# Fabri000/Maze-Solving-Agent-Gymnasium

Measured on NVIDIA B200. Metric: env-steps/sec (40x40 mazes, whole job), higher is better.
Workload: dtype u8/int32 state+obs, f64 reward

## Files before the change

include/maze_b200.h:

```cpp
#ifndef MAZE_B200_H
#define MAZE_B200_H

#include <stdint.h>

#ifdef __cplusplus
extern "C" {
#endif

#define MAZE_ABI_VERSION 12

#define MAZE_E_NULL   (-1)
#define MAZE_E_RANGE  (-2)
#define MAZE_E_SHAPE  (-3)
#define MAZE_E_ALGO   (-4)
#define MAZE_E_ALIGN  (-5)

#define MAZE_MAX_DIM      255
#define MAZE_GEN_MAX_DIM  131
#define MAZE_GEN_MAX_CELLS 64
#define MAZE_WINDOW       15

#define MAZE_ALGO_RPRIM     0
#define MAZE_ALGO_DFS       1
#define MAZE_ALGO_PRIMKILL  2

#define MAZE_META_WORDS 8
#define MAZE_META_H          0
#define MAZE_META_W          1
#define MAZE_META_START      2
#define MAZE_META_GOAL       3
#define MAZE_META_MAX_STEPS  4
#define MAZE_META_FLAGS      5
#define MAZE_META_SOL_LEN    6
#define MAZE_META_SPARE      7
#define MAZE_FLAG_TOROIDAL 1

#define MAZE_TAB_OPEN      0x01
#define MAZE_TAB_CODE_SHIFT 1
#define MAZE_TAB_D4_SHIFT   4

#define MAZE_ST_NEEDS_RESET 0x01
#define MAZE_ST_WON         0x02
#define MAZE_ST_MOVE_SHIFT  2
#define MAZE_ST_NMOVES_SHIFT 4

#define MAZE_STEP_AUTORESET   0x01
#define MAZE_STEP_WIN_NEXT    0x02
#define MAZE_STEP_WIN_QUEUE   0x04
#define MAZE_STEP_PACKED      0x08
#define MAZE_STEP_NO_WIDE     0x10

#define MAZE_REC_CODE_SHIFT   16
#define MAZE_REC_TERM_SHIFT   19
#define MAZE_REC_TRUNC_SHIFT  20
#define MAZE_REC_KIND_SHIFT   21
#define MAZE_REC_INDEX_SHIFT  23
#define MAZE_REC_KIND_REVISIT 0
#define MAZE_REC_KIND_INVALID 1
#define MAZE_REC_KIND_SHAPING 2
#define MAZE_REC_KIND_CONST   3
#define MAZE_REC_CONST_ZERO      0
#define MAZE_REC_CONST_ONE       1
#define MAZE_REC_CONST_MINUS_ONE 2
#define MAZE_REC_REWARD(kind, index) (((uint32_t)(kind) << MAZE_REC_KIND_SHIFT) | ((uint32_t)(index) << MAZE_REC_INDEX_SHIFT))

typedef struct maze_ctx maze_ctx;

typedef struct maze_env_batch {
    int32_t   num_envs;
    int32_t   num_mazes;
    int32_t   slot;
    int32_t   pool_stride;
    const int32_t* meta;
    const uint8_t* table;
    int32_t*  env_maze;
    uint64_t* state;
    uint16_t* visits;
    int32_t*  agent;
    int32_t*  target;
    int32_t*  best_dir;
    double*   reward;
    uint8_t*  terminated;
    uint8_t*  truncated;
    double*   ep_return;
    int64_t*  stats;
    double*   stats_return;
    int32_t*  queue;
    int32_t*  queue_count;
    int64_t   visit_cell_stride;
    int64_t   visit_env_stride;
    int32_t   visit_tiled;
    int32_t   visit_slot;
    int32_t*  target_dirty;
    uint32_t* packed;
    uint32_t* visit_bits;
    int32_t   visit_bits_pitch;
    int32_t   visit_bits_stride;
    int32_t   flags;
    int32_t   reserved;
} maze_env_batch;
#define MAZE_BATCH_BORDERED 1

int  maze_sizeof(int which);

int  maze_abi_version(void);
int  maze_ctx_create(maze_ctx** out, int device);
void maze_ctx_destroy(maze_ctx* ctx);
const char* maze_last_error(maze_ctx* ctx);

int maze_reward_lut(maze_ctx* ctx, int kind, double* out);

int maze_fields(maze_ctx* ctx, const uint8_t* grids, int32_t* meta, uint8_t* table,
                const int32_t* ids, int n, int slot, void* stream);

int maze_step(maze_ctx* ctx, const maze_env_batch* b, const uint8_t* actions, uint32_t mode, void* stream);

int maze_step_decode_host(const uint32_t* records, int64_t n, const int32_t* shape, const uint8_t* toroidal, int32_t* agent,
                          int32_t* best_dir, double* reward, uint8_t* terminated, uint8_t* truncated);

int maze_bench_scatter_rmw(maze_ctx* ctx, const maze_env_batch* b, const uint8_t* actions, uint16_t* arr, int64_t n_elems, int pattern,
                           int rmw_per_1024, uint32_t launch, int streams, void* stream);

typedef struct maze_step_trace {
    int32_t* agent;
    int32_t* best_dir;
    double*  reward;
    uint8_t* terminated;
    uint8_t* truncated;
} maze_step_trace;
int maze_step_many(maze_ctx* ctx, const maze_env_batch* b, const uint8_t* actions, int k_steps, uint32_t mode,
                   const maze_step_trace* trace, int chunk_envs, void* stream);

int maze_reset(maze_ctx* ctx, const maze_env_batch* b, const uint8_t* mask, void* stream);

int maze_generate(maze_ctx* ctx, uint8_t* grids, int32_t* meta, uint8_t* table, const int32_t* ids,
                  const int32_t* count_dev, int n, int slot, int max_h, int max_w,
                  uint64_t seed, int64_t slot_id_base, int candidates, double* difficulty, void* stream);

int maze_curriculum(maze_ctx* ctx, int32_t* meta, int32_t* wins, const int32_t* ids, const int32_t* count_dev,
                    int n, int grow, int max_h, int max_w, int wins_a, int algo_a, int wins_b, int algo_b, void* stream);

int maze_regen_swap(maze_ctx* ctx, uint8_t* grids, uint8_t* table, int32_t* meta, const uint8_t* shadow_grids, const uint8_t* shadow_table,
                    const int32_t* shadow_meta, const int32_t* ready_gen, int depth, const int32_t* queue, const int32_t* queue_count, int n,
                    int slot, int32_t* refill_queue, int32_t* refill_count, int32_t* queued_tag, int batch, int32_t* slow_queue,
                    int32_t* slow_count, int32_t* stats, int32_t* wins, void* stream);
int maze_regen_prepare(maze_ctx* ctx, const int32_t* meta, const int32_t* base_meta, const int32_t* base_wins, int grow, int max_h, int max_w,
                       int wins_a, int algo_a, int wins_b, int algo_b, int32_t* shadow_meta, int32_t* ready_gen, int depth,
                       const int32_t* refill_queue, const int32_t* refill_count, int n, int32_t* work_queue, int32_t* work_count, void* stream);
int maze_regen_publish(maze_ctx* ctx, const int32_t* shadow_meta, int32_t* ready_gen, int depth, const int32_t* work_queue,
                       const int32_t* work_count, int n, void* stream);

int maze_window(maze_ctx* ctx, const maze_env_batch* b, float* window, double* agent_norm, double* target_norm,
                void* stream);

int maze_direction_mask(maze_ctx* ctx, const maze_env_batch* b, int probs, float* mask, void* stream);

#define MAZE_Q_EMPTY     0xffffffffffffffffull
#define MAZE_Q_NO_SLOT   0xffffffffu
typedef struct maze_q_agent {
    int64_t   capacity;
    uint64_t* keys;
    double*   q_a;
    double*   q_b;
    int32_t*  overflow;
    int32_t   envs_per_agent;
    int32_t   eps_len;
    const double* eps_lut;
    double*   gamma;
    double    lr;
    double    eta;
    uint32_t* slot;
    uint32_t* steps_done;
    uint8_t*  last_action;
    double*   ep_return;
    uint64_t  seed;
    int64_t   env_id_base;
    const double*  u_tape;
    const uint8_t* a_tape;
    uint32_t* tape_pos;
    int32_t   u_len, a_len;
} maze_q_agent;

int maze_q_epsilon_lut(double initial_epsilon, double final_epsilon, double decay, double* out, int n);

int maze_q_act(maze_ctx* ctx, const maze_env_batch* b, const maze_q_agent* agent, uint8_t* actions, void* stream);

int maze_q_update(maze_ctx* ctx, const maze_env_batch* b, const maze_q_agent* agent, void* stream);

int maze_q_rollout(maze_ctx* ctx, const maze_env_batch* b, const maze_q_agent* agent, int k_steps, uint32_t mode,
                   void* stream);

#define MAZE_WINDOW_WORDS 24
typedef struct maze_replay {
    int64_t   capacity;
    unsigned long long* pushed;
    float*    vec;
    float*    next_vec;
    uint32_t* win;
    uint32_t* next_win;
    uint8_t*  action;
    float*    reward;
    float*    stage_vec;
    uint32_t* stage_win;
    int32_t   without_replacement;
    int32_t   reserved;
} maze_replay;

int maze_dqn_observe(maze_ctx* ctx, const maze_env_batch* b, const maze_replay* r, void* stream);

int maze_dqn_push(maze_ctx* ctx, const maze_env_batch* b, const maze_replay* r, const uint8_t* actions, void* stream);

int maze_dqn_sample(maze_ctx* ctx, const maze_replay* r, int n, uint64_t seed, uint64_t draw, float* vec, float* win,
                    float* next_vec, float* next_win, int64_t* action, float* reward, void* stream);

int maze_dqn_select(maze_ctx* ctx, const maze_env_batch* b, const float* q_values, const double* eps_lut, int eps_len,
                    uint32_t* steps_done, uint64_t seed, int64_t env_id_base, uint8_t* actions, void* stream);

#define MAZE_NET_IN       1600
#define MAZE_NET_IN_USED  1574
#define MAZE_NET_H1       1024
#define MAZE_NET_H2       512
#define MAZE_NET_OFF_CONV_W 0
#define MAZE_NET_OFF_CONV_B 864
#define MAZE_NET_OFF_W1     896
#define MAZE_NET_OFF_B1     (MAZE_NET_OFF_W1 + MAZE_NET_H1 * MAZE_NET_IN)
#define MAZE_NET_OFF_W2     (MAZE_NET_OFF_B1 + MAZE_NET_H1)
#define MAZE_NET_OFF_B2     (MAZE_NET_OFF_W2 + MAZE_NET_H2 * MAZE_NET_H1)
#define MAZE_NET_OFF_W3     (MAZE_NET_OFF_B2 + MAZE_NET_H2)
#define MAZE_NET_OFF_B3     (MAZE_NET_OFF_W3 + 4 * MAZE_NET_H2)
#define MAZE_NET_PARAMS     (MAZE_NET_OFF_B3 + 4)
typedef struct maze_dqn_net {
    float*    params;
    float*    target;
    float*    grads;
    float*    adam_m;
    float*    adam_v;
    uint16_t* w1_bf16;
    uint16_t* w2_bf16;
    uint16_t* w1t_bf16;
    uint16_t* w2t_bf16;
    uint16_t* tw1_bf16;
    uint16_t* tw2_bf16;
    void*     workspace;
    float*    loss;
    int32_t   max_batch;
    int32_t   reserved;
} maze_dqn_net;

int64_t maze_dqn_net_workspace_bytes(int max_batch);

int maze_dqn_net_refresh(maze_ctx* ctx, const maze_dqn_net* net, int which, void* stream);

int maze_dqn_forward(maze_ctx* ctx, const maze_dqn_net* net, int which, const float* vec, const uint32_t* win, int n,
                     float* q_out, void* stream);

int maze_dqn_features(maze_ctx* ctx, const maze_dqn_net* net, int which, const float* vec, const uint32_t* win, int n,
                      uint16_t* X, uint8_t* pool_idx, void* stream);

int maze_dqn_backward(maze_ctx* ctx, const maze_dqn_net* net, const float* vec, const uint32_t* win, const float* next_vec,
                      const uint32_t* next_win, const uint8_t* action, const float* reward, int n, float gamma,
                      float* qsa_out, void* fc_ready_event, void* stream);

int maze_dqn_adamw(maze_ctx* ctx, const maze_dqn_net* net, float lr, float beta1, float beta2, float eps, float weight_decay,
                   int64_t step, float grad_scale, float clamp, void* stream);

int maze_dqn_net_profile(maze_ctx* ctx, int enable);
int maze_dqn_net_profile_read(maze_ctx* ctx, float* ms, char* labels, int label_bytes, int cap, int* count);

int maze_dqn_sample_packed(maze_ctx* ctx, const maze_replay* r, int n, uint64_t seed, uint64_t draw, float* vec, uint32_t* win,
                           float* next_vec, uint32_t* next_win, uint8_t* action, float* reward, void* stream);

int maze_dqn_gemm_bf16(maze_ctx* ctx, const uint16_t* A, int lda, const uint16_t* B, int ldb, void* C, int ldc, int M, int N, int K,
                       int epilogue, int act, const float* bias, const uint16_t* aux, int ldaux, int tile_n, int splits, void* stream);

#define MAZE_METRIC_WORDS 8
#define MAZE_METRIC_DIFFICULTY 0
#define MAZE_METRIC_COMPLEXITY 1
#define MAZE_METRIC_L          2
#define MAZE_METRIC_DE         3
#define MAZE_METRIC_D          4
#define MAZE_METRIC_SOL_LEN    5
#define MAZE_METRIC_DE_COUNT   6
int maze_difficulty(maze_ctx* ctx, const uint8_t* grids, const int32_t* meta, const int32_t* ids,
                    int n, int slot, int max_h, int max_w, double* out, void* stream);

#define MAZE_METRIC_EXT_WORDS   20
#define MAZE_METRIC_EXT_DENSITY 0
#define MAZE_METRIC_EXT_T       1
#define MAZE_METRIC_EXT_J       2
#define MAZE_METRIC_EXT_CR      3
#define MAZE_METRIC_EXT_AC      4
#define MAZE_METRIC_EXT_FDE     5
#define MAZE_METRIC_EXT_BDE     6
#define MAZE_METRIC_EXT_L_DE    7
#define MAZE_METRIC_EXT_T_DE    8
#define MAZE_METRIC_EXT_D_SHARP 11
#define MAZE_METRIC_EXT_L_SHARP 14
int maze_difficulty_ext(maze_ctx* ctx, const uint8_t* grids, const int32_t* meta, const int32_t* ids,
                        int n, int slot, int max_h, int max_w, double* out, double* ext_out, void* stream);

#define MAZE_RENDER_TILE 16
int maze_render(maze_ctx* ctx, const maze_env_batch* b, const int32_t* env_ids, int n, uint8_t* out,
                int out_h, int out_w, void* stream);

#define MAZE_PACK_BITMAP 0
#define MAZE_PACK_WALLS  1
int maze_pack(maze_ctx* ctx, const uint8_t* grids, const int32_t* meta, const int32_t* ids, int n, int slot,
              int format, uint8_t* packed, int packed_stride, void* stream);
int maze_unpack(maze_ctx* ctx, const uint8_t* packed, int packed_stride, int format, uint8_t* grids,
                const int32_t* meta, const int32_t* ids, int n, int slot, void* stream);

int maze_collection_encode(maze_ctx* ctx, const uint8_t* grids, const int32_t* meta, const int32_t* ids, int n,
                           int slot, int h, int w, int32_t* out, void* stream);

#ifdef __cplusplus
}
#endif
#endif
```

maze-solving-agent-gymnasium_b200/csrc/maze_abi.cu:

```cuda
#include <cmath>
#include <cstdio>
#include <cstdlib>
#include <cstring>
#include <new>
#include "maze_common.cuh"

int maze_fail_cuda(maze_ctx* ctx, cudaError_t e, const char* what) {
    if (ctx) snprintf(ctx->err, sizeof(ctx->err), "CUDA error %d (%s) in %s", (int)e, cudaGetErrorString(e), what);
    return (int)e;
}

int maze_fail_arg(maze_ctx* ctx, int code, const char* what) {
    if (ctx) snprintf(ctx->err, sizeof(ctx->err), "argument error %d: %s", code, what);
    return code;
}

int maze_check_batch(maze_ctx* ctx, const maze_env_batch* b) {
    if (!b) return maze_fail_arg(ctx, MAZE_E_NULL, "batch");
    if (!b->meta || !b->table || !b->env_maze || !b->state || !b->visits || !b->agent || !b->target ||
        !b->best_dir || !b->reward || !b->terminated || !b->truncated)
        return maze_fail_arg(ctx, MAZE_E_NULL, "batch pointer");
    if (b->num_envs <= 0 || b->num_mazes <= 0 || b->slot <= 0 || (b->slot & 1))
        return maze_fail_arg(ctx, MAZE_E_RANGE, "num_envs / num_mazes / slot (must be even)");
    if (b->visit_slot < b->slot || (b->visit_tiled != 0 && b->visit_tiled != 1))
        return maze_fail_arg(ctx, MAZE_E_RANGE, "visit_slot (>= slot) / visit_tiled (0 or 1)");
    if (b->visit_bits && (b->visit_bits_pitch < 1 || b->visit_bits_stride < b->visit_bits_pitch || (b->visit_bits_stride & 3) ||
                          ((uintptr_t)b->visit_bits & 15)))
        return maze_fail_arg(ctx, MAZE_E_RANGE, "visit_bits: pitch >= 1, stride a multiple of 4 words, 16-byte aligned");
    if (b->visit_cell_stride <= 0 || b->visit_env_stride <= 0)
        return maze_fail_arg(ctx, MAZE_E_RANGE, "visit strides (cell-major: B, 1; env-major: 1, slot)");
    if (((uintptr_t)b->meta & 15) || ((uintptr_t)b->state & 7) || ((uintptr_t)b->agent & 7) ||
        ((uintptr_t)b->target & 7) || ((uintptr_t)b->best_dir & 7) || ((uintptr_t)b->reward & 7) ||
        ((uintptr_t)b->visits & 3))
        return maze_fail_arg(ctx, MAZE_E_ALIGN, "batch pointer alignment");
    return 0;
}


extern "C" int maze_abi_version(void) { return MAZE_ABI_VERSION; }

extern "C" int maze_sizeof(int which) {
    switch (which) {
        case 0: return (int)sizeof(maze_env_batch);
        case 1: return (int)sizeof(maze_q_agent);
        case 2: return (int)sizeof(maze_replay);
        case 3: return (int)sizeof(maze_step_trace);
        case 4: return (int)sizeof(maze_dqn_net);
        default: return -1;
    }
}

extern "C" int maze_ctx_create(maze_ctx** out, int device) {
    if (!out) return MAZE_E_NULL;
    *out = nullptr;
    maze_ctx* ctx = new (std::nothrow) maze_ctx();
    if (!ctx) return MAZE_E_RANGE;
    memset(ctx, 0, sizeof(*ctx));
    ctx->device = device;
    for (int i = 0; i < 256; ++i) {
        ctx->h_lut_revisit[i] = 0.0 - (1 - std::exp(-0.2 * i));
        ctx->h_lut_invalid[i] = 0.0 - (1 - std::exp(-0.15 * i));
    }
    ctx->h_shaping[0] = 0 * 0.5 - 0.05;
    ctx->h_shaping[1] = 1 * 0.5 - 0.05;
    ctx->h_shaping[2] = 0.0;
    ctx->h_shaping[3] = -1 * 0.5 - 0.05;
    cudaError_t e = cudaSetDevice(device);
    if (e == cudaSuccess) e = cudaMalloc(&ctx->d_lut_revisit, 256 * sizeof(double));
    if (e == cudaSuccess) e = cudaMalloc(&ctx->d_lut_invalid, 256 * sizeof(double));
    if (e == cudaSuccess) e = cudaMalloc(&ctx->d_counter, 4 * sizeof(int));
    if (e == cudaSuccess) e = cudaMemcpy(ctx->d_lut_revisit, ctx->h_lut_revisit, 256 * sizeof(double), cudaMemcpyHostToDevice);
    if (e == cudaSuccess) e = cudaMemcpy(ctx->d_lut_invalid, ctx->h_lut_invalid, 256 * sizeof(double), cudaMemcpyHostToDevice);
    if (e == cudaSuccess) e = cudaDeviceGetAttribute(&ctx->num_sms, cudaDevAttrMultiProcessorCount, device);
    if (e != cudaSuccess) {
        int rc = (int)e;
        cudaFree(ctx->d_lut_revisit);
        cudaFree(ctx->d_lut_invalid);
        cudaFree(ctx->d_counter);
        delete ctx;
        return rc;
    }
    ctx->step_ept = 2;
    if (const char* v = getenv("MAZE_STEP_EPT")) ctx->step_ept = atoi(v);
    if (const char* v = getenv("MAZE_L2_PERSIST_MB")) {
        int maxp = 0;
        cudaDeviceGetAttribute(&maxp, cudaDevAttrMaxPersistingL2CacheSize, device);
        size_t want = (size_t)atoi(v) << 20, before = 0, after = 0;
        if (want > (size_t)maxp) want = (size_t)maxp;
        cudaDeviceGetLimit(&before, cudaLimitPersistingL2CacheSize);
        cudaError_t le = cudaDeviceSetLimit(cudaLimitPersistingL2CacheSize, want);
        cudaDeviceGetLimit(&after, cudaLimitPersistingL2CacheSize);
        fprintf(stderr, "[maze_b200] persisting L2 %zu -> %zu bytes (max %d, rc %d)\n", before, after, maxp, (int)le);
    }
    if (const char* v = getenv("MAZE_L2_FETCH")) {
        size_t before = 0, after = 0;
        cudaDeviceGetLimit(&before, cudaLimitMaxL2FetchGranularity);
        cudaError_t le = cudaDeviceSetLimit(cudaLimitMaxL2FetchGranularity, (size_t)atoi(v));
        cudaDeviceGetLimit(&after, cudaLimitMaxL2FetchGranularity);
        fprintf(stderr, "[maze_b200] L2 fetch granularity %zu -> %zu (rc %d)\n", before, after, (int)le);
    }
    *out = ctx;
    return 0;
}

extern "C" void maze_ctx_destroy(maze_ctx* ctx) {
    if (!ctx) return;
    cudaFree(ctx->d_lut_revisit);
    cudaFree(ctx->d_lut_invalid);
    cudaFree(ctx->d_counter);
    cudaFree(ctx->d_scratch);
    maze_net_profile_free(ctx);
    delete ctx;
}

extern "C" const char* maze_last_error(maze_ctx* ctx) { return ctx ? ctx->err : "null ctx"; }

extern "C" int maze_reward_lut(maze_ctx* ctx, int kind, double* out) {
    if (!out) return MAZE_E_NULL;
    double rev[256], inv[256];
    for (int i = 0; i < 256; ++i) {
        rev[i] = 0.0 - (1 - std::exp(-0.2 * i));
        inv[i] = 0.0 - (1 - std::exp(-0.15 * i));
    }
    memset(out, 0, 256 * sizeof(double));
    if (kind == 0) memcpy(out, rev, sizeof(rev));
    else if (kind == 1) memcpy(out, inv, sizeof(inv));
    else if (kind == 2) { out[0] = -1 * 0.5 - 0.05; out[1] = 0 * 0.5 - 0.05; out[2] = 1 * 0.5 - 0.05; }
    else return maze_fail_arg(ctx, MAZE_E_RANGE, "maze_reward_lut kind");
    return 0;
}

extern "C" int maze_step_decode_host(const uint32_t* records, int64_t n, const int32_t* shape, const uint8_t* toroidal, int32_t* agent,
                                     int32_t* best_dir, double* reward, uint8_t* terminated, uint8_t* truncated) {
    if (!records || n < 0) return MAZE_E_NULL;
    double lut[4][256];
    memset(lut, 0, sizeof(lut));
    for (int i = 0; i < 256; ++i) {
        lut[MAZE_REC_KIND_REVISIT][i] = 0.0 - (1 - std::exp(-0.2 * i));
        lut[MAZE_REC_KIND_INVALID][i] = 0.0 - (1 - std::exp(-0.15 * i));
    }
    lut[MAZE_REC_KIND_SHAPING][0] = -1 * 0.5 - 0.05;
    lut[MAZE_REC_KIND_SHAPING][1] = 0 * 0.5 - 0.05;
    lut[MAZE_REC_KIND_SHAPING][2] = 1 * 0.5 - 0.05;
    lut[MAZE_REC_KIND_CONST][MAZE_REC_CONST_ONE] = 1.0;
    lut[MAZE_REC_KIND_CONST][MAZE_REC_CONST_MINUS_ONE] = -1.0;
    for (int64_t e = 0; e < n; ++e) {
        const uint32_t rec = records[e];
        const int r = (int)(rec & 0xff), c = (int)((rec >> 8) & 0xff), code = (int)((rec >> MAZE_REC_CODE_SHIFT) & 7);
        if (agent) { agent[2 * e] = r; agent[2 * e + 1] = c; }
        if (best_dir) {
            int br = 0, bc = 0;
            if (code < 4) {
                const int dr = (code == 0) - (code == 1), dc = (code == 2) - (code == 3);
                int nr = r + dr, nc = c + dc;
                if (toroidal && toroidal[e] && shape) {
                    const int H = shape[2 * e], W = shape[2 * e + 1];
                    nr = nr < 0 ? H - 1 : (nr >= H ? 0 : nr);
                    nc = nc < 0 ? W - 1 : (nc >= W ? 0 : nc);
                }
                br = r - nr;
                bc = c - nc;
            }
            best_dir[2 * e] = br;
            best_dir[2 * e + 1] = bc;
        }
        if (reward) reward[e] = lut[(rec >> MAZE_REC_KIND_SHIFT) & 3][(rec >> MAZE_REC_INDEX_SHIFT) & 0xff];
        if (terminated) terminated[e] = (uint8_t)((rec >> MAZE_REC_TERM_SHIFT) & 1);
        if (truncated) truncated[e] = (uint8_t)((rec >> MAZE_REC_TRUNC_SHIFT) & 1);
    }
    return 0;
}
```

maze-solving-agent-gymnasium_b200/csrc/maze_env.cuh:

```cuda
#pragma once
#include "maze_common.cuh"

struct StepLuts {
    const double* revisit;
    const double* invalid;
    double shaping_same, shaping_closer, shaping_farther;
};

inline StepLuts step_luts(const maze_ctx* ctx) {
    StepLuts l;
    l.revisit = ctx->d_lut_revisit;
    l.invalid = ctx->d_lut_invalid;
    l.shaping_same = ctx->h_shaping[0];
    l.shaping_closer = ctx->h_shaping[1];
    l.shaping_farther = ctx->h_shaping[3];
    return l;
}

#define VISIT_AT(b, e, idx) ((b).visits + (size_t)(idx) * (b).visit_cell_stride + (size_t)(e) * (b).visit_env_stride)

#ifndef MAZE_STATE_POLICY
#define MAZE_STATE_POLICY 1
#endif
#ifndef MAZE_TABLE_POLICY
#define MAZE_TABLE_POLICY 1
#endif
#ifndef MAZE_VISIT_POLICY
#define MAZE_VISIT_POLICY 1
#endif

template <int kPolicy>
__device__ __forceinline__ uint64_t l2_policy() {
    uint64_t p = 0;
    if (kPolicy == 1) asm volatile("createpolicy.fractional.L2::evict_last.b64 %0, 1.0;" : "=l"(p));
    if (kPolicy == 2) asm volatile("createpolicy.fractional.L2::evict_first.b64 %0, 1.0;" : "=l"(p));
    return p;
}
template <int kPolicy> __device__ __forceinline__ unsigned long long pol_load(const unsigned long long* p, uint64_t pol) {
    if (kPolicy == 0) return *p;
    unsigned long long v;
    asm volatile("ld.global.L2::cache_hint.u64 %0, [%1], %2;" : "=l"(v) : "l"(p), "l"(pol));
    return v;
}
template <int kPolicy> __device__ __forceinline__ int pol_load(const int* p, uint64_t pol) {
    if (kPolicy == 0) return *p;
    int v;
    asm volatile("ld.global.L2::cache_hint.s32 %0, [%1], %2;" : "=r"(v) : "l"(p), "l"(pol));
    return v;
}
template <int kPolicy> __device__ __forceinline__ unsigned pol_load(const uint16_t* p, uint64_t pol) {
    if (kPolicy == 0) return *p;
    unsigned short v;
    asm volatile("ld.global.L2::cache_hint.u16 %0, [%1], %2;" : "=h"(v) : "l"(p), "l"(pol));
    return v;
}
template <int kPolicy> __device__ __forceinline__ int pol_load_nc(const uint8_t* p, uint64_t pol) {
    if (kPolicy == 0) return __ldg(p);
    unsigned v;
    asm volatile("ld.global.nc.L2::cache_hint.u8 %0, [%1], %2;" : "=r"(v) : "l"(p), "l"(pol));
    return (int)v;
}
template <int kPolicy> __device__ __forceinline__ void pol_store(unsigned long long* p, unsigned long long v, uint64_t pol) {
    if (kPolicy == 0) { *p = v; return; }
    asm volatile("st.global.L2::cache_hint.u64 [%0], %1, %2;" ::"l"(p), "l"(v), "l"(pol) : "memory");
}
template <int kPolicy> __device__ __forceinline__ void pol_store(int* p, int v, uint64_t pol) {
    if (kPolicy == 0) { *p = v; return; }
    asm volatile("st.global.L2::cache_hint.s32 [%0], %1, %2;" ::"l"(p), "r"(v), "l"(pol) : "memory");
}
template <int kPolicy> __device__ __forceinline__ void pol_store(uint16_t* p, unsigned v, uint64_t pol) {
    if (kPolicy == 0) { *p = (uint16_t)v; return; }
    asm volatile("st.global.L2::cache_hint.u16 [%0], %1, %2;" ::"l"(p), "h"((unsigned short)v), "l"(pol) : "memory");
}
__device__ __forceinline__ unsigned visit_load(const uint16_t* p, uint64_t pol) { return pol_load<MAZE_VISIT_POLICY>(p, pol); }
#ifndef MAZE_VISIT_STORE_POLICY
#define MAZE_VISIT_STORE_POLICY MAZE_VISIT_POLICY
#endif
__device__ __forceinline__ void visit_store(uint16_t* p, unsigned v, uint64_t pol) {
    if (MAZE_VISIT_STORE_POLICY == MAZE_VISIT_POLICY) pol_store<MAZE_VISIT_POLICY>(p, v, pol);
    else pol_store<MAZE_VISIT_STORE_POLICY>(p, v, l2_policy<MAZE_VISIT_STORE_POLICY>());
}

__device__ __forceinline__ int visit_index(const maze_env_batch& b, int r, int c, int W) {
    if (b.visit_tiled) return (((r >> 2) * ((W + 3) >> 2) + (c >> 2)) << 4) | ((r & 3) << 2) | (c & 3);
    return r * W + c;
}

__device__ __forceinline__ void visit_bit_set(const maze_env_batch& b, int e, int r, int c) {
    if (b.visit_bits) atomicOr(b.visit_bits + (size_t)e * b.visit_bits_stride + r * b.visit_bits_pitch + (c >> 5), 1u << (c & 31));
}
__device__ __forceinline__ void visit_bits_clear(const maze_env_batch& b, int e) {
    if (!b.visit_bits) return;
    uint4* p = reinterpret_cast<uint4*>(b.visit_bits + (size_t)e * b.visit_bits_stride);
    for (int i = 0; i < (b.visit_bits_stride >> 2); ++i) p[i] = make_uint4(0, 0, 0, 0);
}

__device__ __forceinline__ void warp_clear_visits(unsigned need, const maze_env_batch& b, int e) {
    if (need & (1u << (threadIdx.x & 31)))
        for (int i = 0; i < b.visit_slot; ++i) *VISIT_AT(b, e, i) = 0;
}

__device__ __forceinline__ void begin_episode(EnvState& s, int start, int tab_at_start, bool& wrapped) {
    s.r = start & 0xffff;
    s.c = start >> 16;
    s.consec = 0;
    s.flags = 0;
    s.steps = 0;
    s.epoch += 1;
    wrapped = s.epoch > 255;
    if (wrapped) s.epoch = 1;
    s.tab = tab_at_start;
}

struct MazeView {
    int H, W, start, goal, max_steps;
    bool tor;
    const uint8_t* tab;
};

__device__ __forceinline__ MazeView load_maze(const maze_env_batch& b, int m) {
    const int4* mp = reinterpret_cast<const int4*>(b.meta + (size_t)m * MAZE_META_WORDS);
    const int4 m0 = __ldg(mp), m1 = __ldg(mp + 1);
    MazeView v;
    v.H = m0.x; v.W = m0.y; v.start = m0.z; v.goal = m0.w;
    v.max_steps = m1.x;
    v.tor = (m1.y & MAZE_FLAG_TOROIDAL) != 0;
    v.tab = b.table + (size_t)m * b.slot;
    return v;
}

struct StepResult {
    double reward;
    int term, trunc;
};

__device__ __forceinline__ StepResult env_transition(const maze_env_batch& b, int e, EnvState& st, const MazeView& mz,
                                                     int a, const StepLuts& luts) {
    StepResult out = {0.0, 0, 0};
    int dr, dc;
    action_delta(a, dr, dc);
    int nr = st.r + dr, nc = st.c + dc;
    bool inb = true;
    if (mz.tor) {
        nr = nr < 0 ? mz.H - 1 : (nr >= mz.H ? 0 : nr);
        nc = nc < 0 ? mz.W - 1 : (nc >= mz.W ? 0 : nc);
    } else {
        inb = (nr > 0) & (nr < mz.H - 1) & (nc > 0) & (nc < mz.W - 1);
    }
    const int idx = nr * mz.W + nc;
    const int tb = inb ? __ldg(mz.tab + idx) : 0;
    if (inb && (tb & MAZE_TAB_OPEN)) {
        const uint64_t pol = l2_policy<MAZE_VISIT_POLICY>();
        uint16_t* vp = VISIT_AT(b, e, visit_index(b, nr, nc, mz.W));
        const unsigned vis = visit_load(vp, pol);
        const int cnt = ((int)(vis >> 8) == st.epoch) ? (int)(vis & 0xff) : 0;
        if (cnt == 0) {
            if ((nr | (nc << 16)) == mz.goal) {
                out.reward = 1.0;
                out.term = 1;
            } else {
                const int dd = ((st.tab >> MAZE_TAB_D4_SHIFT) - (tb >> MAZE_TAB_D4_SHIFT)) & 3;
                out.reward = dd == 1 ? luts.shaping_closer : (dd == 3 ? luts.shaping_farther : luts.shaping_same);
            }
        } else {
            out.reward = __ldg(luts.revisit + cnt);
        }
        visit_store(vp, (unsigned)((st.epoch << 8) | (cnt < 255 ? cnt + 1 : 255)), pol);
        visit_bit_set(b, e, nr, nc);
        st.r = nr;
        st.c = nc;
        st.tab = tb;
        st.consec = 0;
        int nm = (st.flags >> MAZE_ST_NMOVES_SHIFT) & 3;
        nm = nm < 2 ? nm + 1 : 2;
        st.flags = (a << MAZE_ST_MOVE_SHIFT) | (nm << MAZE_ST_NMOVES_SHIFT);
    } else {
        st.consec = st.consec < 255 ? st.consec + 1 : 255;
        out.reward = __ldg(luts.invalid + st.consec);
        st.flags &= ~(MAZE_ST_NEEDS_RESET | MAZE_ST_WON);
    }
    st.steps = st.steps < 65535 ? st.steps + 1 : 65535;
    if (st.steps > mz.max_steps) {
        out.trunc = 1;
        out.reward = -1.0;
    }
    if (out.term | out.trunc) st.flags |= MAZE_ST_NEEDS_RESET | (out.term ? MAZE_ST_WON : 0);
    return out;
}
```

maze-solving-agent-gymnasium_b200/csrc/maze_obs.cu:

```cuda
#include "maze_env.cuh"
#include "maze_window.cuh"

namespace {

constexpr int OBS_THREADS = 256;
constexpr int WIN = MAZE_WINDOW;
constexpr int WIN_CELLS = WIN * WIN;

constexpr int WIN_ENVS = OBS_THREADS / 16;
constexpr int WIN_FLOATS = 3 * WIN_CELLS;

#ifndef MAZE_WIN_MINB
#define MAZE_WIN_MINB 4
#endif

__device__ __forceinline__ void window_row_to_smem(uint8_t* sl, unsigned m0, unsigned m1, unsigned m2) {
#pragma unroll
    for (int j = 0; j < WIN; ++j) {
        sl[j] = (uint8_t)((m0 >> j) & 1u);
        sl[WIN_CELLS + j] = (uint8_t)((m1 >> j) & 1u);
        sl[2 * WIN_CELLS + j] = (uint8_t)((m2 >> j) & 1u);
    }
}

__device__ __forceinline__ void window_norms(const EnvState& st, const MazeView& mz, int e, int hl, double* __restrict__ agent_norm,
                                             double* __restrict__ target_norm) {
    if (hl < 2) {
        const double shape = (double)(hl == 0 ? mz.H : mz.W);
        if (agent_norm) agent_norm[(size_t)e * 2 + hl] = __ddiv_rn((double)(hl == 0 ? st.r : st.c), shape);
        if (target_norm) target_norm[(size_t)e * 2 + hl] = __ddiv_rn((double)(hl == 0 ? (mz.goal & 0xffff) : (mz.goal >> 16)), shape);
    }
}

__device__ __forceinline__ void window_stream_out(const uint8_t* s_out, float* __restrict__ out, int n_float) {
    for (int q = threadIdx.x; 4 * q < n_float; q += OBS_THREADS) {
        const int f = 4 * q;
        const unsigned v = *reinterpret_cast<const unsigned*>(s_out + f);
        if (f + 3 < n_float) {
            __stcs(reinterpret_cast<float4*>(out) + q,
                   make_float4(__uint_as_float((v & 1u) * 0x3f800000u), __uint_as_float((v >> 8 & 1u) * 0x3f800000u),
                               __uint_as_float((v >> 16 & 1u) * 0x3f800000u), __uint_as_float((v >> 24 & 1u) * 0x3f800000u)));
        } else {
            for (int i = f; i < n_float; ++i) __stcs(out + i, (float)s_out[i]);
        }
    }
}

__global__ void __launch_bounds__(OBS_THREADS, MAZE_WIN_MINB)
maze_window_kernel(maze_env_batch b, float* __restrict__ window, double* __restrict__ agent_norm,
                   double* __restrict__ target_norm) {
    __shared__ __align__(16) uint8_t s_out[WIN_ENVS * WIN_FLOATS];
    const int hl = threadIdx.x & 15, w = threadIdx.x >> 4;
    const int e0 = blockIdx.x * WIN_ENVS, e = e0 + w;
    if (e < b.num_envs) {
        const EnvState st = unpack_state(b.state[e]);
        const MazeView mz = load_maze(b, b.env_maze[e]);
        unsigned m0, m1, m2;
        window_row_masks(b, e, st, mz, hl, m0, m1, m2);
        if (hl < WIN) window_row_to_smem(s_out + w * WIN_FLOATS + hl * WIN, m0, m1, m2);
        window_norms(st, mz, e, hl, agent_norm, target_norm);
    }
    __syncthreads();
    window_stream_out(s_out, window + (size_t)e0 * WIN_FLOATS, min(WIN_ENVS, b.num_envs - e0) * WIN_FLOATS);
}

constexpr int WINB_PER = 2;
constexpr int WINB_ENVS = WIN_ENVS * WINB_PER;

__global__ void __launch_bounds__(OBS_THREADS, MAZE_WIN_MINB)
maze_window_bordered_kernel(maze_env_batch b, float* __restrict__ window, double* __restrict__ agent_norm,
                            double* __restrict__ target_norm) {
    __shared__ __align__(16) uint8_t s_out[WINB_ENVS * WIN_FLOATS];
    const int hl = threadIdx.x & 15, w = threadIdx.x >> 4;
    const int e0 = blockIdx.x * WINB_ENVS;
    int e[WINB_PER];
    bool valid[WINB_PER];
    uint64_t raw[WINB_PER];
    int maze_id[WINB_PER];
#pragma unroll
    for (int u = 0; u < WINB_PER; ++u) {
        e[u] = e0 + w * WINB_PER + u;
        valid[u] = e[u] < b.num_envs;
        raw[u] = valid[u] ? b.state[e[u]] : 0ull;
        maze_id[u] = valid[u] ? b.env_maze[e[u]] : 0;
    }
    EnvState st[WINB_PER];
    MazeView mz[WINB_PER];
#pragma unroll
    for (int u = 0; u < WINB_PER; ++u) {
        st[u] = unpack_state(raw[u]);
        mz[u] = MazeView{};
        if (valid[u]) mz[u] = load_maze(b, maze_id[u]);
    }
    WindowRowRaw rows[WINB_PER];
    bool has[WINB_PER];
#pragma unroll
    for (int u = 0; u < WINB_PER; ++u) {
        has[u] = valid[u] && hl < WIN && mz[u].H >= WIN && mz[u].W >= WIN;
        rows[u] = WindowRowRaw{};
        if (has[u]) rows[u] = window_row_load_bits(b, e[u], st[u], mz[u], hl);
    }
#pragma unroll
    for (int u = 0; u < WINB_PER; ++u) {
        if (!valid[u]) continue;
        unsigned m0 = 0, m1 = 0, m2 = 0;
        if (has[u]) window_row_fold_bits(rows[u], mz[u], m0, m1, m2);
        if (hl < WIN) window_row_to_smem(s_out + (w * WINB_PER + u) * WIN_FLOATS + hl * WIN, m0, m1, m2);
        window_norms(st[u], mz[u], e[u], hl, agent_norm, target_norm);
    }
    __syncthreads();
    window_stream_out(s_out, window + (size_t)e0 * WIN_FLOATS, min(WINB_ENVS, b.num_envs - e0) * WIN_FLOATS);
}

__global__ void __launch_bounds__(OBS_THREADS)
maze_direction_mask_kernel(maze_env_batch b, int probs, float4* __restrict__ mask) {
    const int e = blockIdx.x * OBS_THREADS + threadIdx.x;
    if (e >= b.num_envs) return;
    const EnvState st = unpack_state(b.state[e]);
    const int m = b.env_maze[e];
    const int2 shape = __ldg(reinterpret_cast<const int2*>(b.meta + (size_t)m * MAZE_META_WORDS));
    const int H = shape.x, W = shape.y;
    const bool tor = (__ldg(b.meta + (size_t)m * MAZE_META_WORDS + MAZE_META_FLAGS) & MAZE_FLAG_TOROIDAL) != 0;
    const uint8_t* tab = b.table + (size_t)m * b.slot;
    float v[4];
#pragma unroll
    for (int a = 0; a < 4; ++a) {
        int dr, dc;
        action_delta(a, dr, dc);
        int nr = st.r + dr, nc = st.c + dc;
        bool open;
        if (tor) {
            nr = nr < 0 ? H - 1 : (nr >= H ? 0 : nr);
            nc = nc < 0 ? W - 1 : (nc >= W ? 0 : nc);
            open = (__ldg(tab + nr * W + nc) & MAZE_TAB_OPEN) != 0;
        } else {
            open = nr >= 0 && nr < H && nc >= 0 && nc < W && (__ldg(tab + nr * W + nc) & MAZE_TAB_OPEN) != 0;
        }
        v[a] = open ? 1.0f : 0.0f;
    }
    if (probs && ((st.flags >> MAZE_ST_NMOVES_SHIFT) & 3) >= 2) {
        const int last = (st.flags >> MAZE_ST_MOVE_SHIFT) & 3;
        const int back = tor ? 3 - last : (last ^ 1);
        v[back] = 0.25f;
    }
    mask[e] = make_float4(v[0], v[1], v[2], v[3]);
}

__global__ void __launch_bounds__(OBS_THREADS)
maze_render_kernel(maze_env_batch b, const int32_t* __restrict__ env_ids, int out_h, int out_w, uint8_t* __restrict__ out) {
    constexpr int T = MAZE_RENDER_TILE;
    const int k = blockIdx.x, r = blockIdx.y;
    const int e = env_ids ? env_ids[k] : k;
    const EnvState st = unpack_state(b.state[e]);
    const int m = b.env_maze[e];
    const int4 m0 = __ldg(reinterpret_cast<const int4*>(b.meta + (size_t)m * MAZE_META_WORDS));
    const int H = m0.x, W = m0.y;
    const int start_r = m0.z & 0xffff, start_c = m0.z >> 16, goal_r = m0.w & 0xffff, goal_c = m0.w >> 16;
    const uint8_t* tab = b.table + (size_t)m * b.slot;
    const bool has_moved = ((st.flags >> MAZE_ST_NMOVES_SHIFT) & 3) >= 1;
    __shared__ uint8_t s_tile[MAZE_GEN_MAX_DIM];
    for (int c = threadIdx.x; c < out_w / T; c += OBS_THREADS) {
        int code = 0;
        if (r < H && c < W) {
            const bool open = (__ldg(tab + r * W + c) & MAZE_TAB_OPEN) != 0;
            const int v = open ? ((r == goal_r && c == goal_c) ? 2 : 1) : 0;
            bool trail = false;
            if (open) {
                const unsigned vis = *VISIT_AT(b, e, visit_index(b, r, c, W));
                const int cnt = ((int)(vis >> 8) == st.epoch) ? (int)(vis & 0xff) : 0;
                if (r == start_r && c == start_c) trail = has_moved;
                else if (r == st.r && c == st.c) trail = cnt >= 2;
                else trail = cnt >= 1;
            }
            code = v | (trail ? 4 : 0) | 8;
        }
        s_tile[c] = (uint8_t)code;
    }
    __syncthreads();
    const int groups = out_w / 4;
    for (int p = threadIdx.x; p < T * groups; p += OBS_THREADS) {
        const int ly = p / groups, x0 = (p % groups) * 4, y = r * T + ly;
        if (y >= out_h) break;
        unsigned char px[12];
#pragma unroll
        for (int i = 0; i < 4; ++i) {
            const int x = x0 + i, c = x / T, lx = x % T;
            const int code = s_tile[c];
            int cr = 0, cg = 0, cb = 0;
            if ((code & 8) && x != W * T - 1 && y != H * T - 1) {
                const int v = code & 3;
                if (lx == 0 || lx == T - 1 || ly == 0 || ly == T - 1) {
                    if (code & 4) { cr = 208; cg = 135; cb = 112; } else { cr = 59; cg = 66; cb = 82; }
                } else if (r == st.r && c == st.c && lx >= T / 4 && lx < T / 4 + T / 2 && ly >= T / 4 && ly < T / 4 + T / 2) {
                    cr = 94; cg = 129; cb = 172;
                } else if (v == 0) { cr = 46; cg = 52; cb = 64; }
                else if (v == 1) { cr = 236; cg = 239; cb = 244; }
                else { cr = 163; cg = 190; cb = 140; }
            }
            px[3 * i] = (unsigned char)cr; px[3 * i + 1] = (unsigned char)cg; px[3 * i + 2] = (unsigned char)cb;
        }
        unsigned* o = reinterpret_cast<unsigned*>(out + (((size_t)k * out_h + y) * out_w + x0) * 3);
#pragma unroll
        for (int w = 0; w < 3; ++w)
            __stcs(o + w, (unsigned)px[4 * w] | ((unsigned)px[4 * w + 1] << 8) | ((unsigned)px[4 * w + 2] << 16) | ((unsigned)px[4 * w + 3] << 24));
    }
}

}

extern "C" int maze_render(maze_ctx* ctx, const maze_env_batch* b, const int32_t* env_ids, int n, uint8_t* out,
                           int out_h, int out_w, void* stream) {
    if (!ctx) return MAZE_E_NULL;
    if (int rc = maze_check_batch(ctx, b)) return rc;
    if (!out) return maze_fail_arg(ctx, MAZE_E_NULL, "maze_render: out");
    if (n <= 0 || out_h <= 0 || out_w <= 0 || out_h % MAZE_RENDER_TILE || out_w % MAZE_RENDER_TILE ||
        out_h / MAZE_RENDER_TILE > MAZE_GEN_MAX_DIM || out_w / MAZE_RENDER_TILE > MAZE_GEN_MAX_DIM)
        return maze_fail_arg(ctx, MAZE_E_RANGE, "maze_render: n / out_h / out_w (multiples of MAZE_RENDER_TILE, at most MAZE_GEN_MAX_DIM tiles)");
    if ((uintptr_t)out & 3) return maze_fail_arg(ctx, MAZE_E_ALIGN, "maze_render: out must be 4-byte aligned");
    if (env_ids == nullptr && n > b->num_envs) return maze_fail_arg(ctx, MAZE_E_RANGE, "maze_render: n exceeds num_envs");
    maze_render_kernel<<<dim3(n, out_h / MAZE_RENDER_TILE), OBS_THREADS, 0, static_cast<cudaStream_t>(stream)>>>(*b, env_ids, out_h, out_w, out);
    MAZE_CHECK(cudaGetLastError());
    return 0;
}

extern "C" int maze_window(maze_ctx* ctx, const maze_env_batch* b, float* window, double* agent_norm,
                           double* target_norm, void* stream) {
    if (!ctx) return MAZE_E_NULL;
    if (int rc = maze_check_batch(ctx, b)) return rc;
    if (!window) return maze_fail_arg(ctx, MAZE_E_NULL, "maze_window: window");
    if (((uintptr_t)window & 15) || ((uintptr_t)agent_norm & 7) || ((uintptr_t)target_norm & 7))
        return maze_fail_arg(ctx, MAZE_E_ALIGN, "maze_window pointer alignment");
    if ((b->flags & MAZE_BATCH_BORDERED) && b->visit_bits) {
        const int grid = (b->num_envs + WINB_ENVS - 1) / WINB_ENVS;
        maze_window_bordered_kernel<<<grid, OBS_THREADS, 0, static_cast<cudaStream_t>(stream)>>>(*b, window, agent_norm, target_norm);
    } else {
        const int grid = (b->num_envs + WIN_ENVS - 1) / WIN_ENVS;
        maze_window_kernel<<<grid, OBS_THREADS, 0, static_cast<cudaStream_t>(stream)>>>(*b, window, agent_norm, target_norm);
    }
    MAZE_CHECK(cudaGetLastError());
    return 0;
}

extern "C" int maze_direction_mask(maze_ctx* ctx, const maze_env_batch* b, int probs, float* mask, void* stream) {
    if (!ctx) return MAZE_E_NULL;
    if (int rc = maze_check_batch(ctx, b)) return rc;
    if (!mask) return maze_fail_arg(ctx, MAZE_E_NULL, "maze_direction_mask: mask");
    if ((uintptr_t)mask & 15) return maze_fail_arg(ctx, MAZE_E_ALIGN, "maze_direction_mask: mask must be 16-byte aligned");
    const int grid = (b->num_envs + OBS_THREADS - 1) / OBS_THREADS;
    maze_direction_mask_kernel<<<grid, OBS_THREADS, 0, static_cast<cudaStream_t>(stream)>>>(
        *b, probs, reinterpret_cast<float4*>(mask));
    MAZE_CHECK(cudaGetLastError());
    return 0;
}
```

maze-solving-agent-gymnasium_b200/csrc/maze_q.cu:

```cuda
#include <cmath>
#include "maze_env.cuh"

namespace {

constexpr int Q_THREADS = 128;
constexpr int Q_MAX_PROBE = 1 << 14;

struct QCursor {
    uint32_t slot, steps_done, pos_u, pos_a;
    double ep_return;
};

__device__ __forceinline__ uint64_t q_key(const EnvState& st, int goal, unsigned agent_id) {
    const unsigned code = ((unsigned)st.tab >> MAZE_TAB_CODE_SHIFT) & 7u;
    return (uint64_t)((unsigned)st.r | ((unsigned)st.c << 8) | ((unsigned)(goal & 0xff) << 16) | ((unsigned)((goal >> 16) & 0xff) << 24)) |
           ((uint64_t)code << 32) | ((uint64_t)agent_id << 35);
}

__device__ __forceinline__ uint32_t q_find_or_insert(const maze_q_agent& ag, uint64_t key) {
    const uint64_t mask = (uint64_t)ag.capacity - 1;
    uint64_t i = (key * 0x9E3779B97F4A7C15ull) >> 20 & mask;
    for (int probe = 0; probe < Q_MAX_PROBE; ++probe) {
        unsigned long long k = *reinterpret_cast<volatile unsigned long long*>(ag.keys + i);
        if (k == key) return (uint32_t)i;
        if (k == MAZE_Q_EMPTY) {
            k = atomicCAS(reinterpret_cast<unsigned long long*>(ag.keys + i), MAZE_Q_EMPTY, (unsigned long long)key);
            if (k == MAZE_Q_EMPTY || k == key) return (uint32_t)i;
        }
        i = (i + 1) & mask;
    }
    *ag.overflow = 1;
    return (uint32_t)(key & mask);
}

__device__ __forceinline__ int argmax4(const double* row) {
    const double2 lo = *reinterpret_cast<const double2*>(row), hi = *reinterpret_cast<const double2*>(row + 2);
    int a = 0;
    double best = lo.x;
    if (lo.y > best) { best = lo.y; a = 1; }
    if (hi.x > best) { best = hi.x; a = 2; }
    if (hi.y > best) { best = hi.y; a = 3; }
    return a;
}

__device__ __forceinline__ double max4(const double* row) {
    const double2 lo = *reinterpret_cast<const double2*>(row), hi = *reinterpret_cast<const double2*>(row + 2);
    return fmax(fmax(lo.x, lo.y), fmax(hi.x, hi.y));
}

__device__ __forceinline__ int q_get_action(const maze_q_agent& ag, int B, int e, QCursor& cur, uint32_t* coin_word) {
    const int li = cur.steps_done < (uint32_t)ag.eps_len ? (int)cur.steps_done : ag.eps_len - 1;
    const double eps = __ldg(ag.eps_lut + li);
    double u;
    uint32_t rnd_action;
    if (ag.u_tape) {
        u = ag.u_tape[(size_t)min(cur.pos_u, (uint32_t)ag.u_len - 1) * B + e];
        ++cur.pos_u;
        rnd_action = 0;
    } else {
        Philox rng;
        rng.init(ag.seed, (uint64_t)(ag.env_id_base + e), cur.steps_done);
        rng.refill();
        u = (double)(((uint64_t)(rng.o0 >> 5) << 26) | (uint64_t)(rng.o1 >> 6)) * (1.0 / 9007199254740992.0);
        rnd_action = rng.o2 >> 30;
        if (coin_word) *coin_word = rng.o3;
    }
    ++cur.steps_done;
    if (u < eps) {
        if (ag.a_tape) {
            rnd_action = ag.a_tape[(size_t)min(cur.pos_a, (uint32_t)ag.a_len - 1) * B + e] & 3u;
            ++cur.pos_a;
        }
        return (int)rnd_action;
    }
    return argmax4(ag.q_a + (size_t)cur.slot * 4);
}

__device__ __forceinline__ void q_learn(const maze_q_agent& ag, int B, int e, QCursor& cur, uint32_t next_slot, int action,
                                        double reward, bool terminated, double gamma) {
    double* row_a = ag.q_a + (size_t)cur.slot * 4;
    if (!ag.q_b) {
        const double future = terminated ? 0.0 : max4(ag.q_a + (size_t)next_slot * 4);
        const double td = __dadd_rn(__dadd_rn(reward, __dmul_rn(gamma, future)), -row_a[action]);
        row_a[action] = __dadd_rn(row_a[action], __dmul_rn(ag.lr, td));
        return;
    }
    bool update_a;
    uint32_t coin = 0;
    if (ag.u_tape) {
        update_a = ag.u_tape[(size_t)min(cur.pos_u, (uint32_t)ag.u_len - 1) * B + e] < 0.5;
        ++cur.pos_u;
    }
    QCursor at_next = cur;
    at_next.slot = next_slot;
    const int best = q_get_action(ag, B, e, at_next, &coin);
    cur.steps_done = at_next.steps_done; cur.pos_u = at_next.pos_u; cur.pos_a = at_next.pos_a;
    if (!ag.u_tape) update_a = (coin >> 31) == 0;
    double* row_b = ag.q_b + (size_t)cur.slot * 4;
    if (update_a) {
        const double boot = ag.q_b[(size_t)next_slot * 4 + best];
        const double td = __dadd_rn(__dadd_rn(reward, __dmul_rn(gamma, boot)), -row_a[action]);
        row_a[action] = __dadd_rn(row_a[action], __dmul_rn(ag.lr, td));
    } else {
        const double boot = ag.q_a[(size_t)next_slot * 4 + best];
        const double td = __dadd_rn(__dadd_rn(reward, __dmul_rn(gamma, boot)), -row_b[action]);
        row_b[action] = __dadd_rn(row_b[action], __dmul_rn(ag.lr, td));
    }
}

__device__ __forceinline__ void q_episode_end(const maze_q_agent& ag, unsigned agent_id, QCursor& cur) {
    const double delta = cur.ep_return > 0.0 ? ag.eta : -ag.eta;
    if (ag.envs_per_agent == 1) ag.gamma[agent_id] = __dadd_rn(ag.gamma[agent_id], delta);
    else atomicAdd(ag.gamma + agent_id, delta / ag.envs_per_agent);
    cur.ep_return = 0.0;
}

__device__ __forceinline__ QCursor load_cursor(const maze_q_agent& ag, int B, int e) {
    QCursor c;
    c.slot = ag.slot[e];
    c.steps_done = ag.steps_done[e];
    c.ep_return = ag.ep_return[e];
    c.pos_u = ag.tape_pos ? ag.tape_pos[e] : 0;
    c.pos_a = ag.tape_pos ? ag.tape_pos[B + e] : 0;
    return c;
}

__device__ __forceinline__ void store_cursor(const maze_q_agent& ag, int B, int e, const QCursor& c) {
    ag.slot[e] = c.slot;
    ag.steps_done[e] = c.steps_done;
    ag.ep_return[e] = c.ep_return;
    if (ag.tape_pos) { ag.tape_pos[e] = c.pos_u; ag.tape_pos[B + e] = c.pos_a; }
}

__global__ void __launch_bounds__(Q_THREADS)
maze_q_act_kernel(maze_env_batch b, maze_q_agent ag, uint8_t* __restrict__ actions) {
    const int e = blockIdx.x * Q_THREADS + threadIdx.x;
    if (e >= b.num_envs) return;
    const EnvState st = unpack_state(b.state[e]);
    if (st.flags & MAZE_ST_NEEDS_RESET) {
        actions[e] = 0;
        ag.last_action[e] = 0;
        return;
    }
    QCursor cur = load_cursor(ag, b.num_envs, e);
    if (cur.slot == MAZE_Q_NO_SLOT) {
        const int goal = __ldg(b.meta + (size_t)b.env_maze[e] * MAZE_META_WORDS + MAZE_META_GOAL);
        cur.slot = q_find_or_insert(ag, q_key(st, goal, (unsigned)(e / ag.envs_per_agent)));
    }
    const int a = q_get_action(ag, b.num_envs, e, cur, nullptr);
    actions[e] = (uint8_t)a;
    ag.last_action[e] = (uint8_t)a;
    store_cursor(ag, b.num_envs, e, cur);
}

__global__ void __launch_bounds__(Q_THREADS)
maze_q_update_kernel(maze_env_batch b, maze_q_agent ag) {
    const int e = blockIdx.x * Q_THREADS + threadIdx.x;
    if (e >= b.num_envs) return;
    const EnvState st = unpack_state(b.state[e]);
    const unsigned agent_id = (unsigned)(e / ag.envs_per_agent);
    const int goal = __ldg(b.meta + (size_t)b.env_maze[e] * MAZE_META_WORDS + MAZE_META_GOAL);
    QCursor cur = load_cursor(ag, b.num_envs, e);
    const uint32_t next_slot = q_find_or_insert(ag, q_key(st, goal, agent_id));
    if (st.steps == 0 || cur.slot == MAZE_Q_NO_SLOT) {
        cur.slot = next_slot;
        store_cursor(ag, b.num_envs, e, cur);
        return;
    }
    const double reward = b.reward[e];
    const bool term = b.terminated[e] != 0, trunc = b.truncated[e] != 0;
    cur.ep_return = __dadd_rn(cur.ep_return, reward);
    q_learn(ag, b.num_envs, e, cur, next_slot, ag.last_action[e] & 3, reward, term, ag.gamma[agent_id]);
    cur.slot = next_slot;
    if (term || trunc) q_episode_end(ag, agent_id, cur);
    store_cursor(ag, b.num_envs, e, cur);
}

__global__ void __launch_bounds__(Q_THREADS)
maze_q_rollout_kernel(maze_env_batch b, maze_q_agent ag, int k_steps, uint32_t mode, StepLuts luts) {
    const int e = blockIdx.x * Q_THREADS + threadIdx.x;
    if (e >= b.num_envs) return;
    const int B = b.num_envs;
    const unsigned agent_id = (unsigned)(e / ag.envs_per_agent);
    EnvState st = unpack_state(b.state[e]);
    int m = b.env_maze[e];
    MazeView mz = load_maze(b, m);
    QCursor cur = load_cursor(ag, B, e);
    double reward = 0.0;
    int term = 0, trunc = 0;
    unsigned long long n_episodes = 0, n_wins = 0, n_steps = 0;
    double return_sum = 0.0;

    for (int k = 0; k < k_steps; ++k) {
        if ((mode & MAZE_STEP_AUTORESET) && (st.flags & MAZE_ST_NEEDS_RESET)) {
            if ((mode & MAZE_STEP_WIN_NEXT) && (st.flags & MAZE_ST_WON)) {
                m += b.pool_stride;
                if (m >= b.num_mazes) m -= b.num_mazes;
                mz = load_maze(b, m);
            }
            bool wrapped;
            begin_episode(st, mz.start, __ldg(mz.tab + (mz.start & 0xffff) * mz.W + (mz.start >> 16)), wrapped);
            visit_bits_clear(b, e);
            if (wrapped)
                for (int i = 0; i < b.visit_slot; ++i) *VISIT_AT(b, e, i) = 0;
            cur.slot = q_find_or_insert(ag, q_key(st, mz.goal, agent_id));
            reward = 0.0; term = 0; trunc = 0;
            continue;
        }
        if (cur.slot == MAZE_Q_NO_SLOT) cur.slot = q_find_or_insert(ag, q_key(st, mz.goal, agent_id));
        const int a = q_get_action(ag, B, e, cur, nullptr);
        const StepResult r = env_transition(b, e, st, mz, a, luts);
        reward = r.reward; term = r.term; trunc = r.trunc;
        ++n_steps;
        const uint32_t next_slot = q_find_or_insert(ag, q_key(st, mz.goal, agent_id));
        cur.ep_return = __dadd_rn(cur.ep_return, reward);
        q_learn(ag, B, e, cur, next_slot, a, reward, term != 0, ag.gamma[agent_id]);
        cur.slot = next_slot;
        if (term | trunc) {
            ++n_episodes;
            n_wins += term;
            return_sum += cur.ep_return;
            q_episode_end(ag, agent_id, cur);
        }
    }

    b.state[e] = pack_state(st);
    b.env_maze[e] = m;
    store_cursor(ag, B, e, cur);
    reinterpret_cast<int2*>(b.agent)[e] = make_int2(st.r, st.c);
    reinterpret_cast<int2*>(b.target)[e] = make_int2(mz.goal & 0xffff, mz.goal >> 16);
    if (b.target_dirty) *b.target_dirty = 1;
    reinterpret_cast<int2*>(b.best_dir)[e] = best_dir_from_code((st.tab >> MAZE_TAB_CODE_SHIFT) & 7, st.r, st.c, mz.H, mz.W, mz.tor);
    b.reward[e] = reward;
    b.terminated[e] = (uint8_t)term;
    b.truncated[e] = (uint8_t)trunc;
    if (b.ep_return) b.ep_return[e] = (term | trunc) ? 0.0 : cur.ep_return;
    if (b.stats && n_steps) atomicAdd(reinterpret_cast<unsigned long long*>(b.stats + 3), n_steps);
    if (b.stats && n_episodes) {
        atomicAdd(reinterpret_cast<unsigned long long*>(b.stats + 0), n_episodes);
        if (n_wins) atomicAdd(reinterpret_cast<unsigned long long*>(b.stats + 1), n_wins);
        if (n_episodes - n_wins) atomicAdd(reinterpret_cast<unsigned long long*>(b.stats + 2), n_episodes - n_wins);
        if (b.stats_return) atomicAdd(b.stats_return, return_sum);
    }
}

int check_agent(maze_ctx* ctx, const maze_env_batch* b, const maze_q_agent* ag) {
    if (!ag) return maze_fail_arg(ctx, MAZE_E_NULL, "q agent");
    if (!ag->keys || !ag->q_a || !ag->overflow || !ag->eps_lut || !ag->gamma || !ag->slot || !ag->steps_done ||
        !ag->last_action || !ag->ep_return)
        return maze_fail_arg(ctx, MAZE_E_NULL, "q agent pointer");
    if (ag->capacity < 16 || (ag->capacity & (ag->capacity - 1)) || ag->capacity > (1ll << 31))
        return maze_fail_arg(ctx, MAZE_E_RANGE, "q agent capacity must be a power of two in [16, 2^31]");
    if (ag->envs_per_agent < 1 || ag->eps_len < 1)
        return maze_fail_arg(ctx, MAZE_E_RANGE, "q agent envs_per_agent / eps_len");
    if ((b->num_envs + ag->envs_per_agent - 1) / ag->envs_per_agent > (1 << 29))
        return maze_fail_arg(ctx, MAZE_E_RANGE, "q agent: more than 2^29 agents");
    if ((ag->u_tape || ag->a_tape) && (!ag->u_tape || !ag->a_tape || !ag->tape_pos || ag->u_len < 1 || ag->a_len < 1))
        return maze_fail_arg(ctx, MAZE_E_NULL, "q agent replay tapes need u_tape, a_tape, tape_pos and lengths");
    if (((uintptr_t)ag->q_a & 31) || ((uintptr_t)ag->q_b & 31) || ((uintptr_t)ag->keys & 7))
        return maze_fail_arg(ctx, MAZE_E_ALIGN, "q agent tables must be 32-byte aligned");
    return 0;
}

}

extern "C" int maze_q_epsilon_lut(double initial_epsilon, double final_epsilon, double decay, double* out, int n) {
    if (!out) return MAZE_E_NULL;
    if (n < 1) return MAZE_E_RANGE;
    for (int i = 0; i < n; ++i)
        out[i] = final_epsilon + (initial_epsilon - final_epsilon) * std::exp(-1. * i / decay);
    return 0;
}

extern "C" int maze_q_act(maze_ctx* ctx, const maze_env_batch* b, const maze_q_agent* agent, uint8_t* actions, void* stream) {
    if (!ctx) return MAZE_E_NULL;
    if (int rc = maze_check_batch(ctx, b)) return rc;
    if (int rc = check_agent(ctx, b, agent)) return rc;
    if (!actions) return maze_fail_arg(ctx, MAZE_E_NULL, "maze_q_act: actions");
    const int grid = (b->num_envs + Q_THREADS - 1) / Q_THREADS;
    maze_q_act_kernel<<<grid, Q_THREADS, 0, static_cast<cudaStream_t>(stream)>>>(*b, *agent, actions);
    MAZE_CHECK(cudaGetLastError());
    return 0;
}

extern "C" int maze_q_update(maze_ctx* ctx, const maze_env_batch* b, const maze_q_agent* agent, void* stream) {
    if (!ctx) return MAZE_E_NULL;
    if (int rc = maze_check_batch(ctx, b)) return rc;
    if (int rc = check_agent(ctx, b, agent)) return rc;
    const int grid = (b->num_envs + Q_THREADS - 1) / Q_THREADS;
    maze_q_update_kernel<<<grid, Q_THREADS, 0, static_cast<cudaStream_t>(stream)>>>(*b, *agent);
    MAZE_CHECK(cudaGetLastError());
    return 0;
}

extern "C" int maze_q_rollout(maze_ctx* ctx, const maze_env_batch* b, const maze_q_agent* agent, int k_steps,
                              uint32_t mode, void* stream) {
    if (!ctx) return MAZE_E_NULL;
    if (int rc = maze_check_batch(ctx, b)) return rc;
    if (int rc = check_agent(ctx, b, agent)) return rc;
    if (k_steps < 1) return maze_fail_arg(ctx, MAZE_E_RANGE, "maze_q_rollout: k_steps");
    if (mode & MAZE_STEP_WIN_QUEUE)
        return maze_fail_arg(ctx, MAZE_E_RANGE, "maze_q_rollout: MAZE_STEP_WIN_QUEUE needs a generation launch between steps; use maze_step");
    const int grid = (b->num_envs + Q_THREADS - 1) / Q_THREADS;
    maze_q_rollout_kernel<<<grid, Q_THREADS, 0, static_cast<cudaStream_t>(stream)>>>(*b, *agent, k_steps, mode, step_luts(ctx));
    MAZE_CHECK(cudaGetLastError());
    return 0;
}
```

maze-solving-agent-gymnasium_b200/csrc/maze_step.cu:

```cuda
#include "maze_env.cuh"

namespace {

constexpr int STEP_THREADS = 256;
#ifndef MAZE_STEP_MINB1
#define MAZE_STEP_MINB1 6
#endif
#ifndef MAZE_STEP_MINB4
#define MAZE_STEP_MINB4 2
#endif
#ifndef MAZE_STEP_MINB2
#define MAZE_STEP_MINB2 5
#endif

template <int EPT, bool kStats, bool kTiled>
__global__ void __launch_bounds__(STEP_THREADS, EPT == 2 ? MAZE_STEP_MINB2 : (EPT == 1 ? MAZE_STEP_MINB1 : MAZE_STEP_MINB4))
maze_step_kernel(maze_env_batch b, const uint8_t* __restrict__ actions, uint32_t mode, StepLuts luts) {
    const int base = blockIdx.x * (STEP_THREADS * EPT) + threadIdx.x;

    const uint64_t pol_state = l2_policy<MAZE_STATE_POLICY>(), pol_table = l2_policy<MAZE_TABLE_POLICY>();
    uint64_t raw[EPT];
    int m[EPT], a[EPT];
    bool valid[EPT];
#pragma unroll
    for (int k = 0; k < EPT; ++k) {
        const int e = base + k * STEP_THREADS;
        valid[k] = e < b.num_envs;
        const int ee = valid[k] ? e : b.num_envs - 1;
        raw[k] = pol_load<MAZE_STATE_POLICY>(reinterpret_cast<const unsigned long long*>(b.state) + ee, pol_state);
        m[k] = pol_load<MAZE_STATE_POLICY>(b.env_maze + ee, pol_state);
        a[k] = __ldcs(actions + ee) & 3;
    }

    bool do_reset[EPT];
    int hw[EPT], tor[EPT];
#pragma unroll
    for (int k = 0; k < EPT; ++k) {
        const int flags = (int)((raw[k] >> 24) & 0xff);
        do_reset[k] = valid[k] && (mode & MAZE_STEP_AUTORESET) && (flags & MAZE_ST_NEEDS_RESET);
        if (do_reset[k] && (mode & MAZE_STEP_WIN_NEXT) && (flags & MAZE_ST_WON)) {
            m[k] += b.pool_stride;
            if (m[k] >= b.num_mazes) m[k] -= b.num_mazes;
            pol_store<MAZE_STATE_POLICY>(b.env_maze + base + k * STEP_THREADS, m[k], pol_state);
        }
        const int2 shape = __ldg(reinterpret_cast<const int2*>(b.meta + (size_t)m[k] * MAZE_META_WORDS));
        hw[k] = shape.x | (shape.y << 16);
        tor[k] = __ldg(b.meta + (size_t)m[k] * MAZE_META_WORDS + MAZE_META_FLAGS) & MAZE_FLAG_TOROIDAL;
    }

    int npos[EPT], idx[EPT], vidx[EPT], tb[EPT];
    bool inb[EPT];
#pragma unroll
    for (int k = 0; k < EPT; ++k) {
        const int H = hw[k] & 0xffff, W = hw[k] >> 16;
        const int r = (int)(raw[k] & 0xff), c = (int)((raw[k] >> 8) & 0xff);
        int dr, dc;
        action_delta(a[k], dr, dc);
        int nr = r + dr, nc = c + dc;
        if (tor[k]) {
            nr = nr < 0 ? H - 1 : (nr >= H ? 0 : nr);
            nc = nc < 0 ? W - 1 : (nc >= W ? 0 : nc);
            inb[k] = true;
        } else {
            inb[k] = (nr > 0) & (nr < H - 1) & (nc > 0) & (nc < W - 1);
        }
        if (do_reset[k]) {
            const int start = __ldg(b.meta + (size_t)m[k] * MAZE_META_WORDS + MAZE_META_START);
            nr = start & 0xffff;
            nc = start >> 16;
            inb[k] = true;
        }
        if (!inb[k]) { nr = r; nc = c; }
        npos[k] = nr | (nc << 16);
        idx[k] = nr * W + nc;
        vidx[k] = kTiled ? ((((nr >> 2) * ((W + 3) >> 2) + (nc >> 2)) << 4) | ((nr & 3) << 2) | (nc & 3)) : idx[k];
#ifdef MAZE_EXP_NOTABLE
        tb[k] = 1 | ((idx[k] & 3) << 1) | ((idx[k] & 3) << 4);
#else
        tb[k] = pol_load_nc<MAZE_TABLE_POLICY>(b.table + (size_t)m[k] * b.slot + idx[k], pol_table);
#endif
    }

    const uint64_t pol = l2_policy<MAZE_VISIT_POLICY>();
    uint32_t vis[EPT];
    bool moved[EPT];
#pragma unroll
    for (int k = 0; k < EPT; ++k) {
        moved[k] = valid[k] && !do_reset[k] && inb[k] && (tb[k] & MAZE_TAB_OPEN);
        vis[k] = 0;
#ifndef MAZE_EXP_NOVISIT
        if (moved[k]) vis[k] = visit_load(VISIT_AT(b, base + k * STEP_THREADS, vidx[k]), pol);
#endif
    }

#pragma unroll
    for (int k = 0; k < EPT; ++k) {
        const int e = base + k * STEP_THREADS;
        const int H = hw[k] & 0xffff, W = hw[k] >> 16;
        const int goal = __ldg(b.meta + (size_t)m[k] * MAZE_META_WORDS + MAZE_META_GOAL);
        const int max_steps = __ldg(b.meta + (size_t)m[k] * MAZE_META_WORDS + MAZE_META_MAX_STEPS);
        double reward = 0.0;
        int term = 0, trunc = 0;
        uint32_t rcode = MAZE_REC_REWARD(MAZE_REC_KIND_CONST, MAZE_REC_CONST_ZERO);
        bool wrapped = false;
        EnvState st = unpack_state(raw[k]);

        if (do_reset[k]) {
            begin_episode(st, npos[k], tb[k], wrapped);
            visit_bits_clear(b, e);
        } else if (valid[k]) {
            if (moved[k]) {
                const int cnt = ((int)(vis[k] >> 8) == st.epoch) ? (int)(vis[k] & 0xff) : 0;
                if (cnt == 0) {
                    if (npos[k] == goal) {
                        reward = 1.0;
                        term = 1;
                        rcode = MAZE_REC_REWARD(MAZE_REC_KIND_CONST, MAZE_REC_CONST_ONE);
                    } else {
                        const int dd = ((st.tab >> MAZE_TAB_D4_SHIFT) - (tb[k] >> MAZE_TAB_D4_SHIFT)) & 3;
                        reward = dd == 1 ? luts.shaping_closer : (dd == 3 ? luts.shaping_farther : luts.shaping_same);
                        rcode = MAZE_REC_REWARD(MAZE_REC_KIND_SHAPING, dd == 1 ? 2u : (dd == 3 ? 0u : 1u));
                    }
                } else {
                    reward = __ldg(luts.revisit + cnt);
                    rcode = MAZE_REC_REWARD(MAZE_REC_KIND_REVISIT, (uint32_t)cnt);
                }
#ifndef MAZE_EXP_NOVISIT
                visit_store(VISIT_AT(b, e, vidx[k]), (unsigned)((st.epoch << 8) | (cnt < 255 ? cnt + 1 : 255)), pol);
                visit_bit_set(b, e, npos[k] & 0xffff, npos[k] >> 16);
#endif
                st.r = npos[k] & 0xffff;
                st.c = npos[k] >> 16;
                st.tab = tb[k];
                st.consec = 0;
                int nm = (st.flags >> MAZE_ST_NMOVES_SHIFT) & 3;
                nm = nm < 2 ? nm + 1 : 2;
                st.flags = (a[k] << MAZE_ST_MOVE_SHIFT) | (nm << MAZE_ST_NMOVES_SHIFT);
            } else {
                st.consec = st.consec < 255 ? st.consec + 1 : 255;
                reward = __ldg(luts.invalid + st.consec);
                rcode = MAZE_REC_REWARD(MAZE_REC_KIND_INVALID, (uint32_t)st.consec);
                st.flags &= ~(MAZE_ST_NEEDS_RESET | MAZE_ST_WON);
            }
            st.steps = st.steps < 65535 ? st.steps + 1 : 65535;
            if (st.steps > max_steps) {
                trunc = 1;
                reward = -1.0;
                rcode = MAZE_REC_REWARD(MAZE_REC_KIND_CONST, MAZE_REC_CONST_MINUS_ONE);
            }
            if (term | trunc) st.flags |= MAZE_ST_NEEDS_RESET | (term ? MAZE_ST_WON : 0);
        }

        const unsigned need = __ballot_sync(0xffffffffu, wrapped);
        if (need) warp_clear_visits(need, b, e);
        if (kStats && b.stats) {
            const unsigned stepped = __ballot_sync(0xffffffffu, valid[k] && !do_reset[k]);
            if (stepped && (threadIdx.x & 31) == 0) atomicAdd(reinterpret_cast<unsigned long long*>(b.stats + 3), (unsigned long long)__popc(stepped));
        }

        if (!valid[k]) continue;

        pol_store<MAZE_STATE_POLICY>(reinterpret_cast<unsigned long long*>(b.state) + e, (unsigned long long)pack_state(st), pol_state);
        if (do_reset[k] && (raw[k] >> 24 & MAZE_ST_WON)) {
            st_cs(reinterpret_cast<int2*>(b.target) + e, make_int2(goal & 0xffff, goal >> 16));
            if (b.target_dirty) *b.target_dirty = 1;
        }
        if (mode & MAZE_STEP_PACKED)
            __stcs(b.packed + e, (uint32_t)st.r | ((uint32_t)st.c << 8) | ((uint32_t)((st.tab >> MAZE_TAB_CODE_SHIFT) & 7) << MAZE_REC_CODE_SHIFT) |
                                     ((uint32_t)term << MAZE_REC_TERM_SHIFT) | ((uint32_t)trunc << MAZE_REC_TRUNC_SHIFT) | rcode);
        if (!(mode & MAZE_STEP_NO_WIDE)) {
            st_cs(reinterpret_cast<int2*>(b.agent) + e, make_int2(st.r, st.c));
            st_cs(reinterpret_cast<int2*>(b.best_dir) + e,
                  best_dir_from_code((st.tab >> MAZE_TAB_CODE_SHIFT) & 7, st.r, st.c, H, W, tor[k] != 0));
            st_cs(b.reward + e, reward);
            __stcs(b.terminated + e, (uint8_t)term);
            __stcs(b.truncated + e, (uint8_t)trunc);
        }

        if (kStats) {
            if (b.ep_return) {
                double g = do_reset[k] ? 0.0 : b.ep_return[e] + reward;
                b.ep_return[e] = g;
                if ((term | trunc) && b.stats_return) atomicAdd(b.stats_return, g);
            }
            if (b.stats) {
                if (term | trunc) {
                    atomicAdd(reinterpret_cast<unsigned long long*>(b.stats + 0), 1ull);
                    if (term) atomicAdd(reinterpret_cast<unsigned long long*>(b.stats + 1), 1ull);
                    else atomicAdd(reinterpret_cast<unsigned long long*>(b.stats + 2), 1ull);
                }
            }
            if (term && (mode & MAZE_STEP_WIN_QUEUE) && b.queue) {
                int at = atomicAdd(b.queue_count, 1);
                b.queue[at] = m[k];
            }
        }
    }
}

__global__ void __launch_bounds__(STEP_THREADS)
maze_reset_kernel(maze_env_batch b, const uint8_t* __restrict__ mask) {
    const int e = blockIdx.x * STEP_THREADS + threadIdx.x;
    const bool valid = e < b.num_envs;
    const int ee = valid ? e : b.num_envs - 1;
    const bool sel = valid && (mask == nullptr || mask[ee] != 0);
    bool wrapped = false;
    EnvState s;
    int H = 0, W = 0, goal = 0;
    bool tor = false;
    if (sel) {
        s = unpack_state(b.state[ee]);
        const int m = b.env_maze[ee];
        const int4* mp = reinterpret_cast<const int4*>(b.meta + (size_t)m * MAZE_META_WORDS);
        const int4 m0 = __ldg(mp);
        const int4 m1 = __ldg(mp + 1);
        H = m0.x; W = m0.y; goal = m0.w;
        tor = (m1.y & MAZE_FLAG_TOROIDAL) != 0;
        const int start = m0.z;
        const int sidx = (start & 0xffff) * W + (start >> 16);
        begin_episode(s, start, __ldg(b.table + (size_t)m * b.slot + sidx), wrapped);
        visit_bits_clear(b, ee);
    }
    const unsigned need = __ballot_sync(0xffffffffu, wrapped);
    if (need) warp_clear_visits(need, b, ee);
    if (!sel) return;
    b.state[e] = pack_state(s);
    reinterpret_cast<int2*>(b.agent)[e] = make_int2(s.r, s.c);
    reinterpret_cast<int2*>(b.target)[e] = make_int2(goal & 0xffff, goal >> 16);
    if (b.target_dirty) *b.target_dirty = 1;
    reinterpret_cast<int2*>(b.best_dir)[e] =
        best_dir_from_code((s.tab >> MAZE_TAB_CODE_SHIFT) & 7, s.r, s.c, H, W, tor);
    b.reward[e] = 0.0;
    b.terminated[e] = 0;
    b.truncated[e] = 0;
    if (b.ep_return) b.ep_return[e] = 0.0;
}

__global__ void __launch_bounds__(STEP_THREADS)
maze_step_many_kernel(maze_env_batch b, const uint8_t* __restrict__ actions, int k_steps, uint32_t mode, StepLuts luts,
                      maze_step_trace tr, int e0, int e1) {
    const int e = e0 + blockIdx.x * STEP_THREADS + threadIdx.x;
    if (e >= e1) return;
    const size_t B = (size_t)b.num_envs;
    EnvState st = unpack_state(b.state[e]);
    int m = b.env_maze[e];
    MazeView mz = load_maze(b, m);
    double reward = 0.0, ep_return = b.ep_return ? b.ep_return[e] : 0.0;
    int term = 0, trunc = 0;
    bool target_changed = false;
    unsigned long long n_episodes = 0, n_wins = 0, n_steps = 0;
    double return_sum = 0.0;
    for (int k = 0; k < k_steps; ++k) {
        if ((mode & MAZE_STEP_AUTORESET) && (st.flags & MAZE_ST_NEEDS_RESET)) {
            if ((mode & MAZE_STEP_WIN_NEXT) && (st.flags & MAZE_ST_WON)) {
                m += b.pool_stride;
                if (m >= b.num_mazes) m -= b.num_mazes;
                mz = load_maze(b, m);
            }
            bool wrapped;
            begin_episode(st, mz.start, __ldg(mz.tab + (mz.start & 0xffff) * mz.W + (mz.start >> 16)), wrapped);
            visit_bits_clear(b, e);
            if (wrapped)
                for (int i = 0; i < b.visit_slot; ++i) *VISIT_AT(b, e, i) = 0;
            reward = 0.0; term = 0; trunc = 0;
            ep_return = 0.0;
            target_changed = true;
        } else {
            const StepResult r = env_transition(b, e, st, mz, __ldcs(actions + (size_t)k * B + e) & 3, luts);
            reward = r.reward; term = r.term; trunc = r.trunc;
            ep_return += reward;
            ++n_steps;
            if (term | trunc) {
                ++n_episodes;
                n_wins += term;
                return_sum += ep_return;
            }
        }
        const size_t at = (size_t)k * B + e;
        if (tr.agent) __stcs(reinterpret_cast<int2*>(tr.agent) + at, make_int2(st.r, st.c));
        if (tr.best_dir)
            __stcs(reinterpret_cast<int2*>(tr.best_dir) + at,
                   best_dir_from_code((st.tab >> MAZE_TAB_CODE_SHIFT) & 7, st.r, st.c, mz.H, mz.W, mz.tor));
        if (tr.reward) __stcs(tr.reward + at, reward);
        if (tr.terminated) __stcs(tr.terminated + at, (uint8_t)term);
        if (tr.truncated) __stcs(tr.truncated + at, (uint8_t)trunc);
    }
    b.state[e] = pack_state(st);
    b.env_maze[e] = m;
    reinterpret_cast<int2*>(b.agent)[e] = make_int2(st.r, st.c);
    if (target_changed) {
        reinterpret_cast<int2*>(b.target)[e] = make_int2(mz.goal & 0xffff, mz.goal >> 16);
        if (b.target_dirty) *b.target_dirty = 1;
    }
    reinterpret_cast<int2*>(b.best_dir)[e] = best_dir_from_code((st.tab >> MAZE_TAB_CODE_SHIFT) & 7, st.r, st.c, mz.H, mz.W, mz.tor);
    b.reward[e] = reward;
    b.terminated[e] = (uint8_t)term;
    b.truncated[e] = (uint8_t)trunc;
    if (b.ep_return) b.ep_return[e] = ep_return;
    if (b.stats && n_steps) atomicAdd(reinterpret_cast<unsigned long long*>(b.stats + 3), n_steps);
    if (n_episodes) {
        if (b.stats) {
            atomicAdd(reinterpret_cast<unsigned long long*>(b.stats + 0), n_episodes);
            if (n_wins) atomicAdd(reinterpret_cast<unsigned long long*>(b.stats + 1), n_wins);
            if (n_episodes - n_wins) atomicAdd(reinterpret_cast<unsigned long long*>(b.stats + 2), n_episodes - n_wins);
        }
        if (b.ep_return && b.stats_return) atomicAdd(b.stats_return, return_sum);
    }
}

}

extern "C" int maze_step_many(maze_ctx* ctx, const maze_env_batch* b, const uint8_t* actions, int k_steps, uint32_t mode,
                              const maze_step_trace* trace, int chunk_envs, void* stream) {
    if (!ctx) return MAZE_E_NULL;
    if (int rc = maze_check_batch(ctx, b)) return rc;
    if (!actions) return maze_fail_arg(ctx, MAZE_E_NULL, "maze_step_many: actions");
    if (k_steps < 1 || chunk_envs < 0) return maze_fail_arg(ctx, MAZE_E_RANGE, "maze_step_many: k_steps / chunk_envs");
    if (mode & MAZE_STEP_WIN_QUEUE)
        return maze_fail_arg(ctx, MAZE_E_RANGE, "maze_step_many: MAZE_STEP_WIN_QUEUE needs a generation launch between steps; use maze_step");
    maze_step_trace tr = {nullptr, nullptr, nullptr, nullptr, nullptr};
    if (trace) tr = *trace;
    if (((uintptr_t)tr.agent & 7) || ((uintptr_t)tr.best_dir & 7) || ((uintptr_t)tr.reward & 7))
        return maze_fail_arg(ctx, MAZE_E_ALIGN, "maze_step_many: trace pointer alignment");
    const int chunk = chunk_envs > 0 ? chunk_envs : b->num_envs;
    const StepLuts luts = step_luts(ctx);
    cudaStream_t st = static_cast<cudaStream_t>(stream);
    for (int e0 = 0; e0 < b->num_envs; e0 += chunk) {
        const int e1 = e0 + chunk < b->num_envs ? e0 + chunk : b->num_envs;
        maze_step_many_kernel<<<(e1 - e0 + STEP_THREADS - 1) / STEP_THREADS, STEP_THREADS, 0, st>>>(*b, actions, k_steps, mode, luts, tr, e0, e1);
    }
    MAZE_CHECK(cudaGetLastError());
    return 0;
}

extern "C" int maze_step(maze_ctx* ctx, const maze_env_batch* b, const uint8_t* actions, uint32_t mode, void* stream) {
    if (!ctx) return MAZE_E_NULL;
    if (int rc = maze_check_batch(ctx, b)) return rc;
    if (!actions) return maze_fail_arg(ctx, MAZE_E_NULL, "actions");
    if ((mode & MAZE_STEP_PACKED) && (!b->packed || ((uintptr_t)b->packed & 3)))
        return maze_fail_arg(ctx, MAZE_E_NULL, "maze_step: MAZE_STEP_PACKED needs batch.packed ([B] uint32)");
    if ((mode & MAZE_STEP_NO_WIDE) && !(mode & MAZE_STEP_PACKED))
        return maze_fail_arg(ctx, MAZE_E_RANGE, "maze_step: MAZE_STEP_NO_WIDE without MAZE_STEP_PACKED would drop the step's outputs");
    const StepLuts luts = step_luts(ctx);
    const bool stats = b->ep_return || b->stats || ((mode & MAZE_STEP_WIN_QUEUE) && b->queue);
    cudaStream_t st = static_cast<cudaStream_t>(stream);
    int ept = ctx->step_ept;
    if (b->num_envs < 64 * 1024) ept = 1;
    auto grid_for = [&](int e) { return (b->num_envs + STEP_THREADS * e - 1) / (STEP_THREADS * e); };
    auto launch = [&](auto kernel, int e) { kernel<<<grid_for(e), STEP_THREADS, 0, st>>>(*b, actions, mode, luts); };
#define MAZE_STEP_DISPATCH(EPT_)                                                                          \
    do {                                                                                                  \
        if (stats) { if (tiled) launch(maze_step_kernel<EPT_, true, true>, EPT_); else launch(maze_step_kernel<EPT_, true, false>, EPT_); } \
        else       { if (tiled) launch(maze_step_kernel<EPT_, false, true>, EPT_); else launch(maze_step_kernel<EPT_, false, false>, EPT_); } \
    } while (0)
    const bool tiled = b->visit_tiled != 0;
    if (ept >= 4) MAZE_STEP_DISPATCH(4);
    else if (ept == 2) MAZE_STEP_DISPATCH(2);
    else MAZE_STEP_DISPATCH(1);
#undef MAZE_STEP_DISPATCH
    MAZE_CHECK(cudaGetLastError());
    return 0;
}

extern "C" int maze_reset(maze_ctx* ctx, const maze_env_batch* b, const uint8_t* mask, void* stream) {
    if (!ctx) return MAZE_E_NULL;
    if (int rc = maze_check_batch(ctx, b)) return rc;
    const int grid = (b->num_envs + STEP_THREADS - 1) / STEP_THREADS;
    maze_reset_kernel<<<grid, STEP_THREADS, 0, static_cast<cudaStream_t>(stream)>>>(*b, mask);
    MAZE_CHECK(cudaGetLastError());
    return 0;
}
```

maze-solving-agent-gymnasium_b200/csrc/maze_window.cuh:

```cuda
#pragma once
#include "maze_env.cuh"

struct WindowRowRaw {
    uint32_t tword[5];
    uint32_t b_lo, b_hi;
    int first, c0;
};

__device__ __forceinline__ WindowRowRaw window_row_load_bits(const maze_env_batch& b, int e, const EnvState& st, const MazeView& mz, int row) {
    constexpr int WIN = MAZE_WINDOW;
    const int r0 = min(max(st.r - WIN / 2, 0), mz.H - WIN), c0 = min(max(st.c - WIN / 2, 0), mz.W - WIN);
    const int rr = r0 + row;
    WindowRowRaw w;
    w.first = rr * mz.W + c0;
    w.c0 = c0;
    const int off = w.first & 3;
    const uint32_t* tw = reinterpret_cast<const uint32_t*>(mz.tab + (w.first - off));
    const uint32_t* brow = b.visit_bits + (size_t)e * b.visit_bits_stride + rr * b.visit_bits_pitch + (c0 >> 5);
#pragma unroll
    for (int k = 0; k < 5; ++k) w.tword[k] = (4 * k - off < WIN) ? __ldg(tw + k) : 0u;
    w.b_lo = brow[0];
    w.b_hi = ((c0 & 31) + WIN > 32) ? brow[1] : 0u;
    return w;
}

__device__ __forceinline__ void window_row_fold_bits(const WindowRowRaw& w, const MazeView& mz, unsigned& m0, unsigned& m1, unsigned& m2) {
    constexpr int WIN = MAZE_WINDOW;
    const int off = w.first & 3;
    const unsigned seen = __funnelshift_r(w.b_lo, w.b_hi, w.c0 & 31) & ((1u << WIN) - 1u);
    unsigned openm = 0;
#pragma unroll
    for (int k = 0; k < 5; ++k)
#pragma unroll
        for (int q = 0; q < 4; ++q) {
            const int jt = 4 * k + q - off;
            if (jt >= 0 && jt < WIN) openm |= ((w.tword[k] >> (8 * q)) & MAZE_TAB_OPEN) << jt;
        }
    const unsigned all = (1u << WIN) - 1u;
    const int start_idx = (mz.start & 0xffff) * mz.W + (mz.start >> 16);
    const int goal_idx = (mz.goal & 0xffff) * mz.W + (mz.goal >> 16);
    const int gj = goal_idx - w.first, sj = start_idx - w.first;
    const unsigned goal_bit = (gj >= 0 && gj < WIN) ? 1u << gj : 0u, start_bit = (sj >= 0 && sj < WIN) ? 1u << sj : 0u;
    m0 = ~openm & all;
    m1 = openm & ~goal_bit;
    m2 = openm & ~start_bit & ~seen;
}

__device__ __forceinline__ void window_row_masks(const maze_env_batch& b, int e, const EnvState& st, const MazeView& mz, int row,
                                                 unsigned& m0, unsigned& m1, unsigned& m2) {
    constexpr int WIN = MAZE_WINDOW;
    m0 = m1 = m2 = 0u;
    const int H = mz.H, W = mz.W;
    if (H < WIN || W < WIN || row >= WIN) return;
    const int start_idx = (mz.start & 0xffff) * W + (mz.start >> 16);
    const int goal_idx = (mz.goal & 0xffff) * W + (mz.goal >> 16);
    int r0 = st.r - WIN / 2, c0 = st.c - WIN / 2;
    if (!mz.tor) {
        r0 = min(max(r0, 0), H - WIN);
        c0 = min(max(c0, 0), W - WIN);
    }
    int rr = r0 + row;
    if (mz.tor) rr = rr < 0 ? rr + H : (rr >= H ? rr - H : rr);
    const uint8_t* trow = mz.tab + rr * W;
    const uint16_t* vbase = b.visits + (size_t)e * b.visit_env_stride;
    const int wt = (W + 3) >> 2;
    if (b.visit_bits && !mz.tor) {
        const WindowRowRaw raw = window_row_load_bits(b, e, st, mz, row);
        window_row_fold_bits(raw, mz, m0, m1, m2);
        return;
    }
    if (!mz.tor && b.visit_tiled && b.visit_cell_stride == 1) {
        const int first = rr * W + c0, off = first & 3;
        const uint32_t* tw = reinterpret_cast<const uint32_t*>(mz.tab + (first - off));
        const int tc0 = c0 >> 2;
        const unsigned long long* vt = reinterpret_cast<const unsigned long long*>(vbase + ((((rr >> 2) * wt) << 4) | ((rr & 3) << 2)));
        uint32_t tword[5];
        unsigned long long vword[5];
#pragma unroll
        for (int k = 0; k < 5; ++k) {
            tword[k] = (4 * k - off < WIN) ? __ldg(tw + k) : 0u;
            vword[k] = (tc0 + k < wt) ? vt[(size_t)(tc0 + k) * 4] : 0ull;
        }
        unsigned openm = 0, seen = 0;
#pragma unroll
        for (int k = 0; k < 5; ++k)
#pragma unroll
            for (int q = 0; q < 4; ++q) {
                const int jt = 4 * k + q - off;
                if (jt >= 0 && jt < WIN) openm |= ((tword[k] >> (8 * q)) & MAZE_TAB_OPEN) << jt;
                const int jv = 4 * (tc0 + k) + q - c0;
                const unsigned v = (unsigned)(vword[k] >> (16 * q)) & 0xffffu;
                if (jv >= 0 && jv < WIN) seen |= (((int)(v >> 8) == st.epoch && (v & 0xffu) != 0) ? 1u : 0u) << jv;
            }
        const unsigned all = (1u << WIN) - 1u;
        const int gj = goal_idx - first, sj = start_idx - first;
        const unsigned goal_bit = (gj >= 0 && gj < WIN) ? 1u << gj : 0u, start_bit = (sj >= 0 && sj < WIN) ? 1u << sj : 0u;
        m0 = ~openm & all;
        m1 = openm & ~goal_bit;
        m2 = openm & ~start_bit & ~seen;
        return;
    }
    const int vrow = b.visit_tiled ? ((((rr >> 2) * wt) << 4) | ((rr & 3) << 2)) : rr * W;
    int tb[WIN];
    unsigned vis[WIN];
#pragma unroll
    for (int j = 0; j < WIN; ++j) {
        int cc = c0 + j;
        if (mz.tor) cc = cc < 0 ? cc + W : (cc >= W ? cc - W : cc);
        tb[j] = __ldg(trow + cc);
        if (b.visit_bits) {
            const uint32_t wv = b.visit_bits[(size_t)e * b.visit_bits_stride + rr * b.visit_bits_pitch + (cc >> 5)];
            vis[j] = ((wv >> (cc & 31)) & 1u) ? (unsigned)((st.epoch << 8) | 1) : 0u;
        } else {
            const int vi = b.visit_tiled ? vrow + (((cc >> 2) << 4) | (cc & 3)) : vrow + cc;
            vis[j] = vbase[(size_t)vi * b.visit_cell_stride];
        }
    }
#pragma unroll
    for (int j = 0; j < WIN; ++j) {
        int cc = c0 + j;
        if (mz.tor) cc = cc < 0 ? cc + W : (cc >= W ? cc - W : cc);
        const int idx = rr * W + cc;
        const bool open = (tb[j] & MAZE_TAB_OPEN) != 0;
        const bool fresh = open && idx != start_idx && !((int)(vis[j] >> 8) == st.epoch && (vis[j] & 0xffu) != 0);
        m0 |= (open ? 0u : 1u) << j;
        m1 |= ((open && idx != goal_idx) ? 1u : 0u) << j;
        m2 |= (fresh ? 1u : 0u) << j;
    }
}
```

maze-solving-agent-gymnasium_b200/maze_b200/cabi.py:

```python
from __future__ import annotations

import ctypes as C
import os

from .build import LIB_PATH

ABI_VERSION = 12
BATCH_BORDERED = 1

META_WORDS = 8
META_H, META_W, META_START, META_GOAL, META_MAX_STEPS, META_FLAGS, META_SOL_LEN, META_SPARE = range(8)
FLAG_TOROIDAL = 1
TAB_OPEN, TAB_CODE_SHIFT, TAB_D4_SHIFT = 0x01, 1, 4
ST_NEEDS_RESET, ST_WON, ST_MOVE_SHIFT, ST_NMOVES_SHIFT = 0x01, 0x02, 2, 4
STEP_AUTORESET, STEP_WIN_NEXT, STEP_WIN_QUEUE, STEP_PACKED, STEP_NO_WIDE = 0x01, 0x02, 0x04, 0x08, 0x10
REC_CODE_SHIFT, REC_TERM_SHIFT, REC_TRUNC_SHIFT, REC_KIND_SHIFT, REC_INDEX_SHIFT = 16, 19, 20, 21, 23
ALGO_RPRIM, ALGO_DFS, ALGO_PRIMKILL = 0, 1, 2
MAX_DIM, GEN_MAX_DIM, WINDOW = 255, 131, 15
METRIC_WORDS = 8
METRIC_NAMES = ("difficulty", "complexity", "L", "DE", "D", "sol_len", "de_count")
PACK_BITMAP, PACK_WALLS = 0, 1
RENDER_TILE = 16
METRIC_EXT_WORDS = 20
METRIC_EXT_NAMES = ("density", "T", "J", "CR", "AC", "FDE", "BDE", "L_DE", "T_DE_AC", "T_DE_FDE", "T_DE_BDE",
                    "D_sharp_AC", "D_sharp_FDE", "D_sharp_BDE", "L_sharp_AC", "L_sharp_FDE", "L_sharp_BDE")
E_NULL, E_RANGE, E_SHAPE, E_ALGO, E_ALIGN = -1, -2, -3, -4, -5


class MazeEnvBatch(C.Structure):
    _fields_ = [
        ("num_envs", C.c_int32), ("num_mazes", C.c_int32), ("slot", C.c_int32), ("pool_stride", C.c_int32),
        ("meta", C.c_void_p), ("table", C.c_void_p), ("env_maze", C.c_void_p), ("state", C.c_void_p),
        ("visits", C.c_void_p), ("agent", C.c_void_p), ("target", C.c_void_p), ("best_dir", C.c_void_p),
        ("reward", C.c_void_p), ("terminated", C.c_void_p), ("truncated", C.c_void_p),
        ("ep_return", C.c_void_p), ("stats", C.c_void_p), ("stats_return", C.c_void_p),
        ("queue", C.c_void_p), ("queue_count", C.c_void_p),
        ("visit_cell_stride", C.c_int64), ("visit_env_stride", C.c_int64),
        ("visit_tiled", C.c_int32), ("visit_slot", C.c_int32),
        ("target_dirty", C.c_void_p), ("packed", C.c_void_p),
        ("visit_bits", C.c_void_p), ("visit_bits_pitch", C.c_int32), ("visit_bits_stride", C.c_int32), ("flags", C.c_int32), ("reserved", C.c_int32),
    ]


class MazeQAgent(C.Structure):
    _fields_ = [
        ("capacity", C.c_int64), ("keys", C.c_void_p), ("q_a", C.c_void_p), ("q_b", C.c_void_p), ("overflow", C.c_void_p),
        ("envs_per_agent", C.c_int32), ("eps_len", C.c_int32), ("eps_lut", C.c_void_p), ("gamma", C.c_void_p),
        ("lr", C.c_double), ("eta", C.c_double),
        ("slot", C.c_void_p), ("steps_done", C.c_void_p), ("last_action", C.c_void_p), ("ep_return", C.c_void_p),
        ("seed", C.c_uint64), ("env_id_base", C.c_int64),
        ("u_tape", C.c_void_p), ("a_tape", C.c_void_p), ("tape_pos", C.c_void_p), ("u_len", C.c_int32), ("a_len", C.c_int32),
    ]


class MazeReplay(C.Structure):
    _fields_ = [
        ("capacity", C.c_int64), ("pushed", C.c_void_p), ("vec", C.c_void_p), ("next_vec", C.c_void_p),
        ("win", C.c_void_p), ("next_win", C.c_void_p), ("action", C.c_void_p), ("reward", C.c_void_p),
        ("stage_vec", C.c_void_p), ("stage_win", C.c_void_p), ("without_replacement", C.c_int32), ("reserved", C.c_int32),
    ]


WINDOW_WORDS = 24
Q_EMPTY = 0xffffffffffffffff
Q_NO_SLOT = 0xffffffff


class MazeStepTrace(C.Structure):
    _fields_ = [("agent", C.c_void_p), ("best_dir", C.c_void_p), ("reward", C.c_void_p), ("terminated", C.c_void_p),
                ("truncated", C.c_void_p)]


class MazeDqnNet(C.Structure):
    _fields_ = [("params", C.c_void_p), ("target", C.c_void_p), ("grads", C.c_void_p), ("adam_m", C.c_void_p), ("adam_v", C.c_void_p),
                ("w1_bf16", C.c_void_p), ("w2_bf16", C.c_void_p), ("w1t_bf16", C.c_void_p), ("w2t_bf16", C.c_void_p),
                ("tw1_bf16", C.c_void_p), ("tw2_bf16", C.c_void_p), ("workspace", C.c_void_p), ("loss", C.c_void_p),
                ("max_batch", C.c_int32), ("reserved", C.c_int32)]


NET_IN, NET_IN_USED, NET_H1, NET_H2 = 1600, 1574, 1024, 512
NET_OFF_CONV_W, NET_OFF_CONV_B, NET_OFF_W1 = 0, 864, 896
NET_OFF_B1 = NET_OFF_W1 + NET_H1 * NET_IN
NET_OFF_W2 = NET_OFF_B1 + NET_H1
NET_OFF_B2 = NET_OFF_W2 + NET_H2 * NET_H1
NET_OFF_W3 = NET_OFF_B2 + NET_H2
NET_OFF_B3 = NET_OFF_W3 + 4 * NET_H2
NET_PARAMS = NET_OFF_B3 + 4


class MazeError(RuntimeError):
    pass


_lib = None

SIGNATURES = {
    "maze_abi_version": (C.c_int, []),
    "maze_ctx_create": (C.c_int, [C.POINTER(C.c_void_p), C.c_int]),
    "maze_ctx_destroy": (None, [C.c_void_p]),
    "maze_last_error": (C.c_char_p, [C.c_void_p]),
    "maze_reward_lut": (C.c_int, [C.c_void_p, C.c_int, C.POINTER(C.c_double)]),
    "maze_fields": (C.c_int, [C.c_void_p, C.c_void_p, C.c_void_p, C.c_void_p, C.c_void_p, C.c_int, C.c_int, C.c_void_p]),
    "maze_step": (C.c_int, [C.c_void_p, C.POINTER(MazeEnvBatch), C.c_void_p, C.c_uint32, C.c_void_p]),
    "maze_step_decode_host": (C.c_int, [C.c_void_p, C.c_int64] + [C.c_void_p] * 7),
    "maze_bench_scatter_rmw": (C.c_int, [C.c_void_p, C.POINTER(MazeEnvBatch), C.c_void_p, C.c_void_p, C.c_int64, C.c_int, C.c_int, C.c_uint32,
                                         C.c_int, C.c_void_p]),
    "maze_step_many": (C.c_int, [C.c_void_p, C.POINTER(MazeEnvBatch), C.c_void_p, C.c_int, C.c_uint32, C.POINTER(MazeStepTrace),
                                 C.c_int, C.c_void_p]),
    "maze_reset": (C.c_int, [C.c_void_p, C.POINTER(MazeEnvBatch), C.c_void_p, C.c_void_p]),
    "maze_generate": (C.c_int, [C.c_void_p, C.c_void_p, C.c_void_p, C.c_void_p, C.c_void_p, C.c_void_p, C.c_int,
                                C.c_int, C.c_int, C.c_int, C.c_uint64, C.c_int64, C.c_int, C.c_void_p, C.c_void_p]),
    "maze_curriculum": (C.c_int, [C.c_void_p, C.c_void_p, C.c_void_p, C.c_void_p, C.c_void_p] + [C.c_int] * 8 + [C.c_void_p]),
    "maze_window": (C.c_int, [C.c_void_p, C.POINTER(MazeEnvBatch), C.c_void_p, C.c_void_p, C.c_void_p, C.c_void_p]),
    "maze_direction_mask": (C.c_int, [C.c_void_p, C.POINTER(MazeEnvBatch), C.c_int, C.c_void_p, C.c_void_p]),
    "maze_q_epsilon_lut": (C.c_int, [C.c_double, C.c_double, C.c_double, C.POINTER(C.c_double), C.c_int]),
    "maze_q_act": (C.c_int, [C.c_void_p, C.POINTER(MazeEnvBatch), C.POINTER(MazeQAgent), C.c_void_p, C.c_void_p]),
    "maze_q_update": (C.c_int, [C.c_void_p, C.POINTER(MazeEnvBatch), C.POINTER(MazeQAgent), C.c_void_p]),
    "maze_q_rollout": (C.c_int, [C.c_void_p, C.POINTER(MazeEnvBatch), C.POINTER(MazeQAgent), C.c_int, C.c_uint32, C.c_void_p]),
    "maze_dqn_observe": (C.c_int, [C.c_void_p, C.POINTER(MazeEnvBatch), C.POINTER(MazeReplay), C.c_void_p]),
    "maze_dqn_push": (C.c_int, [C.c_void_p, C.POINTER(MazeEnvBatch), C.POINTER(MazeReplay), C.c_void_p, C.c_void_p]),
    "maze_dqn_sample": (C.c_int, [C.c_void_p, C.POINTER(MazeReplay), C.c_int, C.c_uint64, C.c_uint64] + [C.c_void_p] * 7),
    "maze_dqn_select": (C.c_int, [C.c_void_p, C.POINTER(MazeEnvBatch), C.c_void_p, C.c_void_p, C.c_int, C.c_void_p,
                                  C.c_uint64, C.c_int64, C.c_void_p, C.c_void_p]),
    "maze_difficulty": (C.c_int, [C.c_void_p, C.c_void_p, C.c_void_p, C.c_void_p, C.c_int, C.c_int, C.c_int, C.c_int,
                                  C.c_void_p, C.c_void_p]),
    "maze_dqn_net_workspace_bytes": (C.c_int64, [C.c_int]),
    "maze_dqn_net_refresh": (C.c_int, [C.c_void_p, C.POINTER(MazeDqnNet), C.c_int, C.c_void_p]),
    "maze_dqn_forward": (C.c_int, [C.c_void_p, C.POINTER(MazeDqnNet), C.c_int, C.c_void_p, C.c_void_p, C.c_int, C.c_void_p, C.c_void_p]),
    "maze_dqn_features": (C.c_int, [C.c_void_p, C.POINTER(MazeDqnNet), C.c_int, C.c_void_p, C.c_void_p, C.c_int, C.c_void_p, C.c_void_p,
                                    C.c_void_p]),
    "maze_dqn_backward": (C.c_int, [C.c_void_p, C.POINTER(MazeDqnNet)] + [C.c_void_p] * 6 + [C.c_int, C.c_float, C.c_void_p, C.c_void_p, C.c_void_p]),
    "maze_dqn_adamw": (C.c_int, [C.c_void_p, C.POINTER(MazeDqnNet)] + [C.c_float] * 5 + [C.c_int64, C.c_float, C.c_float, C.c_void_p]),
    "maze_regen_swap": (C.c_int, [C.c_void_p] + [C.c_void_p] * 7 + [C.c_int] + [C.c_void_p] * 2 + [C.c_int, C.c_int] + [C.c_void_p] * 3 + [C.c_int]
                        + [C.c_void_p] * 5),
    "maze_regen_prepare": (C.c_int, [C.c_void_p] + [C.c_void_p] * 3 + [C.c_int] * 7 + [C.c_void_p] * 2 + [C.c_int] + [C.c_void_p] * 2 + [C.c_int]
                           + [C.c_void_p] * 3),
    "maze_regen_publish": (C.c_int, [C.c_void_p] + [C.c_void_p] * 2 + [C.c_int] + [C.c_void_p] * 2 + [C.c_int, C.c_void_p]),
    "maze_dqn_net_profile": (C.c_int, [C.c_void_p, C.c_int]),
    "maze_dqn_net_profile_read": (C.c_int, [C.c_void_p, C.c_void_p, C.c_void_p, C.c_int, C.c_int, C.POINTER(C.c_int)]),
    "maze_dqn_sample_packed": (C.c_int, [C.c_void_p, C.POINTER(MazeReplay), C.c_int, C.c_uint64, C.c_uint64] + [C.c_void_p] * 7),
    "maze_dqn_gemm_bf16": (C.c_int, [C.c_void_p, C.c_void_p, C.c_int, C.c_void_p, C.c_int, C.c_void_p, C.c_int, C.c_int, C.c_int, C.c_int,
                                     C.c_int, C.c_int, C.c_void_p, C.c_void_p, C.c_int, C.c_int, C.c_int, C.c_void_p]),
    "maze_sizeof": (C.c_int, [C.c_int]),
    "maze_render": (C.c_int, [C.c_void_p, C.POINTER(MazeEnvBatch), C.c_void_p, C.c_int, C.c_void_p, C.c_int, C.c_int, C.c_void_p]),
    "maze_pack": (C.c_int, [C.c_void_p, C.c_void_p, C.c_void_p, C.c_void_p, C.c_int, C.c_int, C.c_int, C.c_void_p, C.c_int,
                            C.c_void_p]),
    "maze_unpack": (C.c_int, [C.c_void_p, C.c_void_p, C.c_int, C.c_int, C.c_void_p, C.c_void_p, C.c_void_p, C.c_int, C.c_int,
                              C.c_void_p]),
    "maze_collection_encode": (C.c_int, [C.c_void_p, C.c_void_p, C.c_void_p, C.c_void_p, C.c_int, C.c_int, C.c_int, C.c_int,
                                         C.c_void_p, C.c_void_p]),
    "maze_difficulty_ext": (C.c_int, [C.c_void_p, C.c_void_p, C.c_void_p, C.c_void_p, C.c_int, C.c_int, C.c_int, C.c_int,
                                  C.c_void_p, C.c_void_p, C.c_void_p]),
}


def lib():
    global _lib
    if _lib is None:
        if not os.path.exists(LIB_PATH):
            raise MazeError(
                f"{LIB_PATH} is missing: build it with `python -c 'import __graft_entry__ as g; g.build()'` "
                "(nvcc, sm_100a).  This package has no CPU or PyTorch fallback.")
        l = C.CDLL(LIB_PATH)
        for name, (res, args) in SIGNATURES.items():
            fn = getattr(l, name)
            fn.restype, fn.argtypes = res, args
        if l.maze_abi_version() != ABI_VERSION:
            raise MazeError(f"ABI mismatch: library {l.maze_abi_version()} vs binding {ABI_VERSION}; rebuild")
        _lib = l
    return _lib


class Context:

    _by_device: dict = {}

    def __init__(self, device_index: int):
        self.device_index = int(device_index)
        self._h = C.c_void_p()
        rc = lib().maze_ctx_create(C.byref(self._h), self.device_index)
        if rc != 0:
            raise MazeError(f"maze_ctx_create(device={device_index}) failed with code {rc} "
                            "(a CUDA device is required; there is no CPU fallback)")

    @classmethod
    def for_device(cls, device) -> "Context":
        import torch
        dev = torch.device(device)
        if dev.type != "cuda":
            raise MazeError(f"device {dev} is not CUDA: the maze kernels are sm_100a only, there is no CPU path")
        idx = dev.index if dev.index is not None else torch.cuda.current_device()
        if idx not in cls._by_device:
            cls._by_device[idx] = cls(idx)
        return cls._by_device[idx]

    @property
    def handle(self):
        return self._h

    def check(self, rc: int, what: str):
        if rc != 0:
            msg = lib().maze_last_error(self._h)
            raise MazeError(f"{what} failed ({rc}): {msg.decode() if msg else ''}")


def reward_lut(kind: int):
    import numpy as np
    out = (C.c_double * 256)()
    rc = lib().maze_reward_lut(None, kind, out)
    if rc != 0:
        raise MazeError(f"maze_reward_lut({kind}) -> {rc}")
    return np.array(out, dtype=np.float64)


def reward_table():
    import numpy as np
    t = np.zeros((4, 256), dtype=np.float64)
    t[0], t[1] = reward_lut(0), reward_lut(1)
    t[2, :3] = reward_lut(2)[:3]
    t[3, :3] = (0.0, 1.0, -1.0)
    return t


def decode_records(records, shape=None, toroidal=None):
    import numpy as np
    rec = np.ascontiguousarray(records).view(np.uint32).reshape(-1)
    n = rec.shape[0]
    out = dict(agent=np.empty((n, 2), np.int32), best_dir=np.empty((n, 2), np.int32), reward=np.empty(n, np.float64),
               terminated=np.empty(n, np.uint8), truncated=np.empty(n, np.uint8))
    sh = None if shape is None else np.ascontiguousarray(shape, dtype=np.int32)
    to = None if toroidal is None else np.ascontiguousarray(toroidal, dtype=np.uint8)
    rc = lib().maze_step_decode_host(rec.ctypes.data, n, None if sh is None else sh.ctypes.data, None if to is None else to.ctypes.data,
                                     out["agent"].ctypes.data, out["best_dir"].ctypes.data, out["reward"].ctypes.data,
                                     out["terminated"].ctypes.data, out["truncated"].ctypes.data)
    if rc != 0:
        raise MazeError(f"maze_step_decode_host -> {rc}")
    out["terminated"], out["truncated"] = out["terminated"].view(np.bool_), out["truncated"].view(np.bool_)
    return out


def ptr(t):
    return None if t is None else C.c_void_p(t.data_ptr())


def current_stream(device):
    import torch
    return C.c_void_p(torch.cuda.current_stream(device).cuda_stream)
```

maze-solving-agent-gymnasium_b200/maze_b200/engine.py:

```python
from __future__ import annotations

import ctypes as C
from typing import Optional, Sequence

import numpy as np
import torch

from . import cabi

ALGO_IDS = {"r-prim": cabi.ALGO_RPRIM, "dfs": cabi.ALGO_DFS, "prim&kill": cabi.ALGO_PRIMKILL}
ALGO_NAMES = {v: k for k, v in ALGO_IDS.items()}


def _round_up(x: int, m: int) -> int:
    return (x + m - 1) // m * m


def check_shape(shape, limit=cabi.MAX_DIM):
    H, W = int(shape[0]), int(shape[1])
    if H % 2 == 0 or W % 2 == 0:
        raise ValueError(f"maze block shape must be odd (2N+1), got {(H, W)}")
    if H < 5 or W < 5 or H > limit or W > limit:
        raise ValueError(f"maze block shape {(H, W)} outside [5, {limit}]")
    return H, W


class MazePool:

    def __init__(self, num_mazes: int, max_shape, device="cuda"):
        self.device = torch.device(device)
        self.ctx = cabi.Context.for_device(self.device)
        self.max_shape = check_shape(max_shape)
        self.num_mazes = int(num_mazes)
        self.slot = _round_up(self.max_shape[0] * self.max_shape[1], 16)
        d = self.device
        self.grids = torch.zeros((self.num_mazes, self.slot), dtype=torch.uint8, device=d)
        self.table = torch.zeros((self.num_mazes, self.slot), dtype=torch.uint8, device=d)
        self.meta = torch.zeros((self.num_mazes, cabi.META_WORDS), dtype=torch.int32, device=d)
        self.any_toroidal = False

    @classmethod
    def from_grids(cls, grids: Sequence[np.ndarray], starts, goals, toroidal, device="cuda", max_shape=None):
        M = len(grids)
        tor = [bool(toroidal)] * M if isinstance(toroidal, (bool, int)) else [bool(t) for t in toroidal]
        shapes = [np.asarray(g).shape for g in grids]
        if max_shape is None:
            max_shape = (max(s[0] for s in shapes), max(s[1] for s in shapes))
        pool = cls(M, max_shape, device)
        pool.upload(range(M), grids, starts, goals, tor)
        return pool

    def upload(self, ids, grids, starts, goals, toroidal):
        ids = list(ids)
        hg = np.zeros((len(ids), self.slot), dtype=np.uint8)
        hm = np.zeros((len(ids), cabi.META_WORDS), dtype=np.int32)
        toroidal = list(toroidal)
        self.any_toroidal = self.any_toroidal or any(bool(t) for t in toroidal)
        for k, (g, s, t, tor) in enumerate(zip(grids, starts, goals, toroidal)):
            g = np.asarray(g, dtype=np.uint8)
            H, W = check_shape(g.shape)
            if H * W > self.slot:
                raise ValueError(f"maze {g.shape} does not fit slot of {self.slot} bytes")
            hg[k, :H * W] = g.reshape(-1)
            hg[k, int(t[0]) * W + int(t[1])] = 2
            hm[k, cabi.META_H], hm[k, cabi.META_W] = H, W
            hm[k, cabi.META_START] = int(s[0]) | (int(s[1]) << 16)
            hm[k, cabi.META_GOAL] = int(t[0]) | (int(t[1]) << 16)
            hm[k, cabi.META_FLAGS] = cabi.FLAG_TOROIDAL if tor else 0
        idx = torch.as_tensor(ids, dtype=torch.long, device=self.device)
        self.grids[idx] = torch.from_numpy(hg).to(self.device)
        self.meta[idx] = torch.from_numpy(hm).to(self.device)
        self.compute_fields(ids)

    def compute_fields(self, ids=None):
        if ids is None:
            ids_t, n = None, self.num_mazes
        else:
            ids_t = torch.as_tensor(list(ids), dtype=torch.int32, device=self.device)
            n = ids_t.numel()
        rc = cabi.lib().maze_fields(self.ctx.handle, cabi.ptr(self.grids), cabi.ptr(self.meta), cabi.ptr(self.table),
                                    cabi.ptr(ids_t), n, self.slot, cabi.current_stream(self.device))
        self.ctx.check(rc, "maze_fields")

    def generate(self, ids=None, shapes=None, algorithms="r-prim", toroidal=False, seed=0, slot_id_base=0,
                 count_dev=None, configure=True, candidates=1, difficulty_out=None):
        if ids is None:
            ids_list = list(range(self.num_mazes))
            ids_t = None
        elif isinstance(ids, torch.Tensor):
            ids_list, ids_t = None, ids.to(device=self.device, dtype=torch.int32).contiguous()
        else:
            ids_list = [int(i) for i in ids]
            ids_t = torch.as_tensor(ids_list, dtype=torch.int32, device=self.device)
        n = self.num_mazes if ids_t is None else ids_t.numel()
        max_h, max_w = self.max_shape
        if configure:
            assert ids_list is not None
            k = len(ids_list)
            if shapes is None:
                shapes = self.max_shape
            def record(shape, a, t):
                H, W = check_shape(shape, cabi.GEN_MAX_DIM - 2 - (2 if t else 0))
                if H * W > self.slot:
                    raise ValueError(f"shape {(H, W)} does not fit the pool slot")
                if isinstance(a, str):
                    if a not in ALGO_IDS:
                        raise ValueError(f"unknown maze generation algorithm {a!r} (expected one of {list(ALGO_IDS)})")
                    a = ALGO_IDS[a]
                elif a not in ALGO_NAMES:
                    raise ValueError(f"unknown maze generation algorithm id {a}")
                return (H, W, (cabi.FLAG_TOROIDAL if t else 0) | (int(a) << 8))

            uniform = (isinstance(shapes[0], (int, np.integer)) and isinstance(algorithms, (str, int))
                       and isinstance(toroidal, (bool, int)))
            if uniform:
                hm = np.tile(np.array(record(shapes, algorithms, toroidal), dtype=np.int32), (k, 1))
            else:
                shp = [shapes] * k if isinstance(shapes[0], (int, np.integer)) else list(shapes)
                alg = [algorithms] * k if isinstance(algorithms, (str, int)) else list(algorithms)
                tor = [toroidal] * k if isinstance(toroidal, (bool, int)) else list(toroidal)
                cache = {}
                hm = np.zeros((k, 3), dtype=np.int32)
                for q in range(k):
                    key = (tuple(shp[q]), alg[q], bool(tor[q]))
                    if key not in cache:
                        cache[key] = record(*key)
                    hm[q] = cache[key]
            some_tor = bool((hm[:, 2] & cabi.FLAG_TOROIDAL).any())
            self.any_toroidal = some_tor if len(ids_list) == self.num_mazes and len(set(ids_list)) == self.num_mazes else (self.any_toroidal or some_tor)
            cfg = torch.from_numpy(hm).to(self.device)
            idx = torch.as_tensor(ids_list, dtype=torch.long, device=self.device)
            self.meta[idx, cabi.META_H] = cfg[:, 0]
            self.meta[idx, cabi.META_W] = cfg[:, 1]
            self.meta[idx, cabi.META_FLAGS] = cfg[:, 2]
        rc = cabi.lib().maze_generate(self.ctx.handle, cabi.ptr(self.grids), cabi.ptr(self.meta), cabi.ptr(self.table),
                                      cabi.ptr(ids_t), cabi.ptr(count_dev), n, self.slot, max_h, max_w,
                                      int(seed) & (2**64 - 1), int(slot_id_base), int(candidates),
                                      cabi.ptr(difficulty_out), cabi.current_stream(self.device))
        self.ctx.check(rc, "maze_generate")

    def curriculum(self, ids, count_dev, wins: torch.Tensor, grow: int = 0, schedule=((5, "prim&kill"), (10, "dfs"))):
        sched = list(schedule or ())
        (wa, aa), (wb, ab) = (sched + [(0, None), (0, None)])[:2]
        code = lambda a: -1 if a is None else (ALGO_IDS[a] if isinstance(a, str) else int(a))
        ids_t = ids.to(device=self.device, dtype=torch.int32).contiguous()
        rc = cabi.lib().maze_curriculum(self.ctx.handle, cabi.ptr(self.meta), cabi.ptr(wins), cabi.ptr(ids_t), cabi.ptr(count_dev),
                                        ids_t.numel(), int(grow), self.max_shape[0], self.max_shape[1], int(wa), code(aa),
                                        int(wb), code(ab), cabi.current_stream(self.device))
        self.ctx.check(rc, "maze_curriculum")

    def difficulty(self, ids=None, extended: bool = False):
        if ids is None:
            ids_t, n = None, self.num_mazes
        else:
            ids_t = torch.as_tensor(ids, dtype=torch.int32, device=self.device).contiguous()
            n = ids_t.numel()
        out = torch.empty((n, cabi.METRIC_WORDS), dtype=torch.float64, device=self.device)
        if extended:
            ext = torch.empty((n, cabi.METRIC_EXT_WORDS), dtype=torch.float64, device=self.device)
            rc = cabi.lib().maze_difficulty_ext(self.ctx.handle, cabi.ptr(self.grids), cabi.ptr(self.meta), cabi.ptr(ids_t), n,
                                                self.slot, self.max_shape[0], self.max_shape[1], cabi.ptr(out), cabi.ptr(ext),
                                                cabi.current_stream(self.device))
            self.ctx.check(rc, "maze_difficulty_ext")
            return out, ext
        rc = cabi.lib().maze_difficulty(self.ctx.handle, cabi.ptr(self.grids), cabi.ptr(self.meta), cabi.ptr(ids_t), n,
                                        self.slot, self.max_shape[0], self.max_shape[1], cabi.ptr(out),
                                        cabi.current_stream(self.device))
        self.ctx.check(rc, "maze_difficulty")
        return out

    def state_dict(self):
        return {"max_shape": tuple(self.max_shape), "grids": self.grids, "table": self.table, "meta": self.meta}

    def load_state_dict(self, sd):
        if tuple(sd["max_shape"]) != tuple(self.max_shape) or sd["grids"].shape != self.grids.shape:
            raise ValueError("checkpoint was taken from a pool of another size / shape")
        for k in ("grids", "table", "meta"):
            getattr(self, k).copy_(sd[k])
        self.any_toroidal = bool((self.meta[:, cabi.META_FLAGS] & cabi.FLAG_TOROIDAL).any().item())

    def meta_host(self):
        return self.meta.cpu().numpy()

    def grid_host(self, m: int) -> np.ndarray:
        mh = self.meta[m].cpu().numpy()
        H, W = int(mh[cabi.META_H]), int(mh[cabi.META_W])
        return self.grids[m, :H * W].cpu().numpy().reshape(H, W)

    def table_host(self, m: int) -> np.ndarray:
        mh = self.meta[m].cpu().numpy()
        H, W = int(mh[cabi.META_H]), int(mh[cabi.META_W])
        return self.table[m, :H * W].cpu().numpy().reshape(H, W)


class MazeBatch:

    def __init__(self, pool: MazePool, num_envs: int, env_maze=None, stats: bool = False, pool_stride: int = 1,
                 queue: bool = False, visit_layout: str = "cell", visit_bits: bool = False):
        if visit_layout not in ("cell", "env", "tile"):
            raise ValueError("visit_layout must be 'cell', 'env' or 'tile'")
        self.visit_layout = visit_layout
        self.pool = pool
        self.device = pool.device
        self.ctx = pool.ctx
        B = self.num_envs = int(num_envs)
        d = self.device
        if env_maze is None:
            env_maze = torch.arange(B, dtype=torch.int32, device=d) % pool.num_mazes
        self.env_maze = torch.as_tensor(env_maze, dtype=torch.int32, device=d).contiguous()
        assert self.env_maze.shape == (B,)
        self.state = torch.zeros(B, dtype=torch.int64, device=d)
        mh, mw = pool.max_shape
        self.visit_slot = pool.slot if visit_layout != "tile" else _round_up(16 * ((mh + 3) // 4) * ((mw + 3) // 4), 16)
        self.visits = torch.zeros((self.visit_slot, B) if visit_layout == "cell" else (B, self.visit_slot),
                                  dtype=torch.int16, device=d)
        self.window = None
        self.agent_norm = None
        self.target_norm = None
        self.dir_mask = None
        self.agent = torch.zeros((B, 2), dtype=torch.int32, device=d)
        self.target = torch.zeros((B, 2), dtype=torch.int32, device=d)
        self.best_dir = torch.zeros((B, 2), dtype=torch.int32, device=d)
        self.reward = torch.zeros(B, dtype=torch.float64, device=d)
        self.terminated = torch.zeros(B, dtype=torch.uint8, device=d)
        self.truncated = torch.zeros(B, dtype=torch.uint8, device=d)
        self.ep_return = torch.zeros(B, dtype=torch.float64, device=d) if stats else None
        self.stats = torch.zeros(4, dtype=torch.int64, device=d) if stats else None
        self.stats_return = torch.zeros(1, dtype=torch.float64, device=d) if stats else None
        self.queue = torch.zeros(B, dtype=torch.int32, device=d) if queue else None
        self.queue_count = torch.zeros(1, dtype=torch.int32, device=d) if queue else None
        self.target_dirty = torch.zeros(1, dtype=torch.int32, device=d)
        self.packed = torch.zeros(B, dtype=torch.int32, device=d)
        self.visit_bits_pitch = (mw + 31) // 32
        self.visit_bits_stride = _round_up(mh * self.visit_bits_pitch, 4)
        self.visit_bits = torch.zeros((B, self.visit_bits_stride), dtype=torch.int32, device=d) if visit_bits else None
        self.pool_stride = int(pool_stride)
        self._c = self._make_struct()

    _CKPT = ("env_maze", "state", "visits", "agent", "target", "best_dir", "reward", "terminated", "truncated",
             "ep_return", "stats", "stats_return", "queue", "queue_count", "target_dirty", "visit_bits")

    def state_dict(self):
        sd = {k: getattr(self, k) for k in self._CKPT if getattr(self, k) is not None}
        sd["visit_layout"] = self.visit_layout
        return sd

    def load_state_dict(self, sd):
        if sd["visit_layout"] != self.visit_layout or sd["state"].shape != self.state.shape:
            raise ValueError("checkpoint was taken from a batch of another size / visit layout")
        for k in self._CKPT:
            if getattr(self, k) is not None and k in sd:
                getattr(self, k).copy_(sd[k])
        self.target_dirty.fill_(1)

    def _make_struct(self) -> cabi.MazeEnvBatch:
        p = self.pool
        return cabi.MazeEnvBatch(
            num_envs=self.num_envs, num_mazes=p.num_mazes, slot=p.slot, pool_stride=self.pool_stride,
            meta=p.meta.data_ptr(), table=p.table.data_ptr(), env_maze=self.env_maze.data_ptr(),
            state=self.state.data_ptr(), visits=self.visits.data_ptr(), agent=self.agent.data_ptr(),
            target=self.target.data_ptr(), best_dir=self.best_dir.data_ptr(), reward=self.reward.data_ptr(),
            terminated=self.terminated.data_ptr(), truncated=self.truncated.data_ptr(),
            ep_return=None if self.ep_return is None else self.ep_return.data_ptr(),
            stats=None if self.stats is None else self.stats.data_ptr(),
            stats_return=None if self.stats_return is None else self.stats_return.data_ptr(),
            queue=None if self.queue is None else self.queue.data_ptr(),
            queue_count=None if self.queue_count is None else self.queue_count.data_ptr(),
            visit_cell_stride=self.num_envs if self.visit_layout == "cell" else 1,
            visit_env_stride=1 if self.visit_layout == "cell" else self.visit_slot,
            visit_tiled=1 if self.visit_layout == "tile" else 0, visit_slot=self.visit_slot,
            target_dirty=self.target_dirty.data_ptr(), packed=self.packed.data_ptr(),
            visit_bits=None if self.visit_bits is None else self.visit_bits.data_ptr(),
            visit_bits_pitch=self.visit_bits_pitch, visit_bits_stride=self.visit_bits_stride,
            flags=0 if p.any_toroidal else cabi.BATCH_BORDERED, reserved=0)

    def sync_flags(self):
        want = 0 if self.pool.any_toroidal else cabi.BATCH_BORDERED
        if self._c.flags != want:
            self._c.flags = want

    def view_struct(self, lo: int, hi: int) -> cabi.MazeEnvBatch:
        if not 0 <= lo < hi <= self.num_envs:
            raise ValueError("env range outside the batch")
        c = cabi.MazeEnvBatch.from_buffer_copy(self._c)
        c.num_envs = hi - lo
        for name, per_env_bytes in (("env_maze", 4), ("state", 8), ("agent", 8), ("target", 8), ("best_dir", 8), ("reward", 8),
                                    ("terminated", 1), ("truncated", 1), ("ep_return", 8), ("packed", 4)):
            base = getattr(self._c, name)
            if base:
                setattr(c, name, base + lo * per_env_bytes)
        c.visits = self._c.visits + lo * self._c.visit_env_stride * 2
        if self._c.visit_bits:
            c.visit_bits = self._c.visit_bits + lo * self.visit_bits_stride * 4
        return c

    def step_view(self, view: cabi.MazeEnvBatch, actions_ptr, mode: int, stream):
        rc = cabi.lib().maze_step(self.ctx.handle, C.byref(view), actions_ptr, mode, stream)
        self.ctx.check(rc, "maze_step")

    def reset(self, mask: Optional[torch.Tensor] = None):
        if mask is not None:
            mask = mask.to(device=self.device, dtype=torch.uint8).contiguous()
        rc = cabi.lib().maze_reset(self.ctx.handle, C.byref(self._c), cabi.ptr(mask), cabi.current_stream(self.device))
        self.ctx.check(rc, "maze_reset")

    def step(self, actions: torch.Tensor, mode: int = 0):
        if actions.dtype != torch.uint8 or actions.device != self.device or not actions.is_contiguous():
            actions = actions.to(device=self.device, dtype=torch.uint8).contiguous()
        assert actions.numel() == self.num_envs
        rc = cabi.lib().maze_step(self.ctx.handle, C.byref(self._c), cabi.ptr(actions), mode,
                                  cabi.current_stream(self.device))
        self.ctx.check(rc, "maze_step")

    def step_many(self, actions: torch.Tensor, mode: int = 0, trace: bool = False, chunk_envs: int = 0):
        if actions.dtype != torch.uint8 or actions.device != self.device or not actions.is_contiguous():
            actions = actions.to(device=self.device, dtype=torch.uint8).contiguous()
        K = actions.shape[0]
        assert actions.shape == (K, self.num_envs)
        out, tr = None, None
        if trace:
            d, B = self.device, self.num_envs
            out = dict(agent=torch.empty((K, B, 2), dtype=torch.int32, device=d), best_dir=torch.empty((K, B, 2), dtype=torch.int32, device=d),
                       reward=torch.empty((K, B), dtype=torch.float64, device=d), terminated=torch.empty((K, B), dtype=torch.uint8, device=d),
                       truncated=torch.empty((K, B), dtype=torch.uint8, device=d))
            tr = cabi.MazeStepTrace(**{k: v.data_ptr() for k, v in out.items()})
        rc = cabi.lib().maze_step_many(self.ctx.handle, C.byref(self._c), cabi.ptr(actions), int(K), int(mode),
                                       C.byref(tr) if tr is not None else None, int(chunk_envs), cabi.current_stream(self.device))
        self.ctx.check(rc, "maze_step_many")
        return out

    def compute_window(self):
        if self.window is None:
            d, B = self.device, self.num_envs
            self.window = torch.empty((B, 3, cabi.WINDOW, cabi.WINDOW), dtype=torch.float32, device=d)
            self.agent_norm = torch.empty((B, 2), dtype=torch.float64, device=d)
            self.target_norm = torch.empty((B, 2), dtype=torch.float64, device=d)
        self.sync_flags()
        rc = cabi.lib().maze_window(self.ctx.handle, C.byref(self._c), cabi.ptr(self.window), cabi.ptr(self.agent_norm),
                                    cabi.ptr(self.target_norm), cabi.current_stream(self.device))
        self.ctx.check(rc, "maze_window")
        return self.window

    def render(self, env_ids=None) -> torch.Tensor:
        ids_t = None if env_ids is None else torch.as_tensor(list(env_ids), dtype=torch.int32, device=self.device)
        n = self.num_envs if ids_t is None else ids_t.numel()
        H, W = self.pool.max_shape
        out = torch.empty((n, H * cabi.RENDER_TILE, W * cabi.RENDER_TILE, 3), dtype=torch.uint8, device=self.device)
        rc = cabi.lib().maze_render(self.ctx.handle, C.byref(self._c), cabi.ptr(ids_t), n, cabi.ptr(out), out.shape[1], out.shape[2],
                                    cabi.current_stream(self.device))
        self.ctx.check(rc, "maze_render")
        return out

    def direction_mask(self, probs: bool = False):
        if self.dir_mask is None:
            self.dir_mask = torch.empty((self.num_envs, 4), dtype=torch.float32, device=self.device)
        rc = cabi.lib().maze_direction_mask(self.ctx.handle, C.byref(self._c), int(bool(probs)), cabi.ptr(self.dir_mask),
                                            cabi.current_stream(self.device))
        self.ctx.check(rc, "maze_direction_mask")
        return self.dir_mask

    def state_host(self):
        s = self.state.cpu().numpy().view(np.uint64)
        return dict(r=(s & 0xff).astype(int), c=((s >> 8) & 0xff).astype(int), consec=((s >> 16) & 0xff).astype(int),
                    flags=((s >> 24) & 0xff).astype(int), steps=((s >> 32) & 0xffff).astype(int),
                    epoch=((s >> 48) & 0xff).astype(int), tab=((s >> 56) & 0xff).astype(int))
```

maze-solving-agent-gymnasium_b200/maze_b200/vector_env.py:

```python
from __future__ import annotations

from types import SimpleNamespace
from typing import Optional

import os

import numpy as np
import torch

from . import cabi
from .engine import ALGO_IDS, MazeBatch, MazePool

from . import _gym as _gymshim

_gym = None
if _gymshim.HAVE_GYMNASIUM:
    import gymnasium as _gym
_VectorBase = _gymshim.VectorEnv


class _LazyInfo(dict):

    def __init__(self, env):
        super().__init__()
        self._env = env

    def __missing__(self, key):
        if key == "distance":
            b = self._env.batch
            v = (b.agent - b.target).abs().sum(dim=1).to(torch.float64)
            self[key] = v
            return v
        raise KeyError(key)

    def __contains__(self, key):
        return key == "distance" or super().__contains__(key)


class _ActionSpace:
    def __init__(self, n, num_envs=None, seed=None):
        self.n = n
        self._num = num_envs
        self._rng = np.random.default_rng(seed)

    def sample(self):
        if self._num is None:
            return int(self._rng.integers(self.n))
        return self._rng.integers(0, self.n, size=self._num).astype(np.uint8)


class MazeVectorEnv(_VectorBase):
    def __init__(self, num_envs: int, shape=(81, 81), topology: str = "euclid", algorithms="r-prim",
                 num_mazes: Optional[int] = None, device="cuda", seed: int = 0, autoreset: bool = True,
                 on_win: str = "keep", reference_order: bool = False, stats: bool = True,
                 slot_id_base: int = 0, pool: Optional[MazePool] = None, env_maze=None, enrich: bool = False,
                 candidates: int = 1, start_shape=None, grow: int = 0, algorithm_schedule=None, visit_layout=None,
                 regenerate_ahead: Optional[int] = None):
        if topology not in ("euclid", "toroidal"):
            raise ValueError("topology must be 'euclid' or 'toroidal'")
        if on_win not in ("keep", "next", "regenerate"):
            raise ValueError("on_win must be 'keep', 'next' or 'regenerate'")
        self.num_envs = int(num_envs)
        self.device = torch.device(device)
        self.topology = topology
        self.shape = (int(shape[0]), int(shape[1]))
        self.seed = int(seed)
        self.autoreset = bool(autoreset)
        self.on_win = on_win
        self.reference_order = bool(reference_order)
        self.slot_id_base = int(slot_id_base)
        self.enrich = bool(enrich)
        self.candidates = int(candidates)
        if self.enrich and self.shape[0] != self.shape[1]:
            raise ValueError("the enriched observation needs square mazes: the reference clamps the window's columns with the "
                             "row count (lib/maze_handler.py:21-29)")
        if self.enrich and min(self.shape) < cabi.WINDOW:
            raise ValueError(f"the enriched observation needs mazes of at least {cabi.WINDOW} x {cabi.WINDOW} blocks")
        if pool is None:
            M = self.num_envs if num_mazes is None else int(num_mazes)
            pool = MazePool(M, self.shape, self.device)
            algos = algorithms
            if not isinstance(algorithms, str):
                algos = [algorithms[i % len(algorithms)] for i in range(M)]
            shapes0 = self.shape if start_shape is None else start_shape
            if not isinstance(shapes0[0], (int, np.integer)):
                shapes0 = [tuple(shapes0[i % len(shapes0)]) for i in range(M)]
            pool.generate(shapes=shapes0, algorithms=algos, toroidal=(topology == "toroidal"),
                          seed=self.seed, slot_id_base=self.slot_id_base, candidates=self.candidates)
        self.pool = pool
        if on_win == "regenerate" and pool.num_mazes != self.num_envs:
            raise ValueError("on_win='regenerate' needs one maze slot per env (num_mazes == num_envs)")
        self.grow = int(grow)
        self.algorithm_schedule = tuple(algorithm_schedule) if algorithm_schedule else ()
        if (self.grow or self.algorithm_schedule) and on_win != "regenerate":
            raise ValueError("grow / algorithm_schedule act when a maze is regenerated: use on_win='regenerate'")
        self.wins = torch.zeros(pool.num_mazes, dtype=torch.int32, device=self.device)
        if regenerate_ahead is None:
            regenerate_ahead = int(os.environ.get("MAZE_REGEN_AHEAD", "3") or 0)
        self.regenerate_depth = min(8, int(regenerate_ahead))
        self.regenerate_ahead = self.regenerate_depth > 0 and on_win == "regenerate"
        self._ahead = None
        if env_maze is None:
            per = max(1, self.num_envs // pool.num_mazes)
            env_maze = (torch.arange(self.num_envs, device=self.device, dtype=torch.int32) // per).clamp_(max=pool.num_mazes - 1)
        self.batch = MazeBatch(pool, self.num_envs, env_maze=env_maze, stats=stats, queue=(on_win == "regenerate"),
                               visit_layout=visit_layout or ("tile" if self.enrich else "cell"), visit_bits=self.enrich)
        self._mode = ((cabi.STEP_AUTORESET if self.autoreset else 0)
                      | (cabi.STEP_WIN_NEXT if on_win == "next" else 0)
                      | (cabi.STEP_WIN_QUEUE if on_win == "regenerate" else 0))
        sp = _gymshim.spaces
        hi = max(self.pool.max_shape)
        if self.enrich:
            single = {"agent": sp.Box(0.0, 1.0, shape=(2,), dtype=np.float64), "target": sp.Box(0.0, 1.0, shape=(2,), dtype=np.float64),
                      "best dir": sp.Box(-hi, hi, shape=(2,), dtype=np.int32),
                      "window": sp.Box(0.0, 1.0, shape=(3, cabi.WINDOW, cabi.WINDOW), dtype=np.float32)}
        else:
            single = {"agent": sp.Box(0, hi, shape=(2,), dtype=np.int32), "target": sp.Box(0, hi, shape=(2,), dtype=np.int32),
                      "best dir": sp.Box(-hi, hi, shape=(2,), dtype=np.int32)}
        self.single_observation_space = sp.Dict(single)
        self.observation_space = sp.Dict({k: sp.Box(v.low if np.isscalar(v.low) else float(np.min(v.low)), v.high if np.isscalar(v.high) else float(np.max(v.high)),
                                                    shape=(self.num_envs,) + tuple(v.shape), dtype=v.dtype) for k, v in single.items()})
        if _gym is not None:
            self.single_action_space = sp.Discrete(4)
            self.action_space = sp.MultiDiscrete([4] * self.num_envs)
        else:
            self.single_action_space = _ActionSpace(4)
            self.action_space = _ActionSpace(4, self.num_envs, seed)
        self._h_actions = None
        self._d_actions = torch.zeros(self.num_envs, dtype=torch.uint8, device=self.device)
        self._h_out = None
        self._h_flag = None
        self._h_packed = None
        self._h_shape_valid = False
        shapes = self.pool.meta[:, :2]
        self._pool_is_uniform = bool((shapes == shapes[0]).all().item()) and not self.grow
        self._h_bytes, self._h_calls = 0, 0

    def _obs(self):
        b = self.batch
        if self.enrich:
            b.compute_window()
            return {"agent": b.agent_norm, "target": b.target_norm, "best dir": b.best_dir, "window": b.window}
        return {"agent": b.agent, "target": b.target, "best dir": b.best_dir}

    def step_many(self, actions, trace: bool = True):
        if self.on_win == "regenerate":
            raise cabi.MazeError("step_many cannot regenerate mazes between its fused steps")
        return self.batch.step_many(actions, self._mode, trace=trace)

    def get_mask_direction(self, probs: bool = False):
        return self.batch.direction_mask(probs)

    def reset(self, seed: Optional[int] = None, options: Optional[dict] = None):
        self.batch.reset()
        return self._obs(), _LazyInfo(self)

    def _device_actions(self, actions):
        if isinstance(actions, torch.Tensor):
            if actions.device == self.device and actions.dtype == torch.uint8 and actions.is_contiguous():
                return actions
            self._d_actions.copy_(actions.reshape(-1), non_blocking=True)
            return self._d_actions
        a = np.ascontiguousarray(actions, dtype=np.uint8).reshape(-1)
        if self._h_actions is None:
            self._h_actions = torch.empty(self.num_envs, dtype=torch.uint8, pin_memory=True)
        self._h_actions.numpy()[:] = a
        self._d_actions.copy_(self._h_actions, non_blocking=True)
        return self._d_actions

    def drain_regeneration(self):
        b = self.batch
        if self.regenerate_ahead:
            return self._drain_ahead()
        if self.grow or self.algorithm_schedule:
            self.pool.curriculum(b.queue, b.queue_count, self.wins, self.grow, self.algorithm_schedule)
        self.pool.generate(ids=b.queue, count_dev=b.queue_count, configure=False, seed=self.seed,
                           slot_id_base=self.slot_id_base, candidates=self.candidates)
        b.queue_count.zero_()

    def _curriculum_rule(self):
        sched = list(self.algorithm_schedule or ())
        (wa, aa), (wb, ab) = (sched + [(0, None), (0, None)])[:2]
        code = lambda a: -1 if a is None else (ALGO_IDS[a] if isinstance(a, str) else int(a))
        return (int(self.grow), self.pool.max_shape[0], self.pool.max_shape[1], int(wa), code(aa), int(wb), code(ab))

    def _build_ahead(self):
        pool, dev, M, K = self.pool, self.device, self.pool.num_mazes, self.regenerate_depth
        idx = dev.index if dev.index is not None else torch.cuda.current_device()
        i32 = dict(dtype=torch.int32, device=dev)
        grids = torch.zeros((K, M, pool.slot), dtype=torch.uint8, device=dev)
        table = torch.zeros((K, M, pool.slot), dtype=torch.uint8, device=dev)
        meta = torch.zeros((K, M, cabi.META_WORDS), **i32)
        ctx = cabi.Context(idx)
        ring = []
        for j in range(K):
            sh = MazePool.__new__(MazePool)
            sh.device, sh.ctx, sh.max_shape, sh.num_mazes, sh.slot = dev, ctx, pool.max_shape, M, pool.slot
            sh.grids, sh.table, sh.meta, sh.any_toroidal = grids[j], table[j], meta[j], pool.any_toroidal
            ring.append(sh)
        curriculum = bool(self.grow or self.algorithm_schedule)
        a = SimpleNamespace(ring=ring, grids=grids, table=table, meta=meta, ctx=ctx, ready=torch.zeros((K, M), **i32),
                 base_meta=pool.meta.clone(), base_wins=self.wins.clone() if curriculum else None, curriculum=curriculum,
                 refill=[torch.arange(M, **i32), torch.zeros(M, **i32)], refill_count=[torch.full((1,), M, **i32), torch.zeros(1, **i32)],
                 tag=torch.full((M,), -1, **i32), slow=torch.zeros(M, **i32), slow_count=torch.zeros(1, **i32),
                 work=torch.zeros((K, M), **i32), work_count=torch.zeros(K, **i32), stats=torch.zeros(2, **i32),
                 side=torch.cuda.Stream(device=dev), side_done=torch.cuda.Event(), main_evt=torch.cuda.Event(), cur=0, batch=0, jobs=0)
        self._ahead = a
        self._refill_job(0)
        for t in (grids, table, meta, a.ready, *a.refill, *a.refill_count, a.work, a.work_count, pool.meta, a.base_meta):
            t.record_stream(a.side)
        if a.base_wins is not None:
            a.base_wins.record_stream(a.side)

    def _refill_job(self, cur):
        a, pool, K = self._ahead, self.pool, self.regenerate_depth
        lib, p, ctx, M = cabi.lib(), cabi.ptr, a.ctx, pool.num_mazes
        stream = cabi.current_stream(self.device)
        rc = lib.maze_regen_prepare(ctx.handle, p(pool.meta), p(a.base_meta), p(a.base_wins), *self._curriculum_rule(), p(a.meta),
                                    p(a.ready), K, p(a.refill[cur]), p(a.refill_count[cur]), M, p(a.work), p(a.work_count), stream)
        ctx.check(rc, "maze_regen_prepare")
        for j, sh in enumerate(a.ring):
            sh.generate(ids=a.work[j], count_dev=a.work_count[j:j + 1], configure=False, seed=self.seed, slot_id_base=self.slot_id_base,
                        candidates=self.candidates)
        rc = lib.maze_regen_publish(ctx.handle, p(a.meta), p(a.ready), K, p(a.work), p(a.work_count), M, stream)
        ctx.check(rc, "maze_regen_publish")
        a.refill_count[cur].zero_()
        a.work_count.zero_()

    def _fit_ahead_depth(self):
        per_entry = self.pool.num_mazes * (2 * self.pool.slot + 4 * cabi.META_WORDS + 4)
        free, _ = torch.cuda.mem_get_info(self.device)
        depth = self.regenerate_depth
        while depth > 0 and depth * per_entry > free // 2:
            depth -= 1
        if depth != self.regenerate_depth:
            import warnings
            warnings.warn(f"regenerate_ahead={self.regenerate_depth} needs {self.regenerate_depth * per_entry / 2**30:.1f} GiB for {self.pool.num_mazes} maze slots; "
                          f"using depth {depth}" + (" (regeneration in place)" if depth == 0 else ""))
            self.regenerate_depth = depth
            self.regenerate_ahead = depth > 0
        return self.regenerate_ahead

    def _drain_ahead(self):
        if self._ahead is None:
            if not self._fit_ahead_depth():
                return self.drain_regeneration()
            self._build_ahead()
        a, b, pool, K = self._ahead, self.batch, self.pool, self.regenerate_depth
        cur, M = a.cur, pool.num_mazes
        lib, p = cabi.lib(), cabi.ptr
        a.slow_count.zero_()
        rc = lib.maze_regen_swap(pool.ctx.handle, p(pool.grids), p(pool.table), p(pool.meta), p(a.grids), p(a.table), p(a.meta), p(a.ready), K,
                                 p(b.queue), p(b.queue_count), M, pool.slot, p(a.refill[cur]), p(a.refill_count[cur]), p(a.tag), a.batch,
                                 p(a.slow), p(a.slow_count), p(a.stats), p(self.wins) if a.curriculum else None,
                                 cabi.current_stream(self.device))
        pool.ctx.check(rc, "maze_regen_swap")
        if a.curriculum:
            pool.curriculum(a.slow, a.slow_count, self.wins, self.grow, self.algorithm_schedule)
        pool.generate(ids=a.slow, count_dev=a.slow_count, configure=False, seed=self.seed, slot_id_base=self.slot_id_base,
                      candidates=self.candidates)
        b.queue_count.zero_()
        if a.side_done.query():
            main, side = torch.cuda.current_stream(self.device), a.side
            a.main_evt.record(main)
            side.wait_event(a.main_evt)
            with torch.cuda.stream(side):
                self._refill_job(cur)
                a.side_done.record(side)
            a.cur, a.batch, a.jobs = cur ^ 1, a.batch + 1, a.jobs + 1

    def regeneration_statistics(self):
        if self._ahead is None:
            return (0, 0, 0)
        fast, slow = (int(v) for v in self._ahead.stats.tolist())
        return (fast, slow, self._ahead.jobs)

    def _drop_ahead(self):
        if self._ahead is not None:
            self._ahead.side.synchronize()
            self._ahead = None

    def step(self, actions, extra_mode: int = 0, observe: bool = True):
        b = self.batch
        if self.on_win == "regenerate":
            self.drain_regeneration()
        b.step(self._device_actions(actions), self._mode | extra_mode)
        term, trunc = b.terminated.view(torch.bool), b.truncated.view(torch.bool)
        if not observe:
            return (None, b.reward, trunc, term, None) if self.reference_order else (None, b.reward, term, trunc, None)
        if self.reference_order:
            return self._obs(), b.reward, trunc, term, _LazyInfo(self)
        return self._obs(), b.reward, term, trunc, _LazyInfo(self)

    def _host_out(self):
        if self._h_out is None:
            B = self.num_envs
            pin = dict(pin_memory=True)
            self._h_out = dict(agent=torch.empty((B, 2), dtype=torch.int32, **pin),
                               target=torch.empty((B, 2), dtype=torch.int32, **pin),
                               best_dir=torch.empty((B, 2), dtype=torch.int32, **pin),
                               reward=torch.empty(B, dtype=torch.float64, **pin),
                               terminated=torch.empty(B, dtype=torch.uint8, **pin),
                               truncated=torch.empty(B, dtype=torch.uint8, **pin))
            if self.enrich:
                self._h_out.update(window=torch.empty((B, 3, cabi.WINDOW, cabi.WINDOW), dtype=torch.float32, **pin),
                                   agent_norm=torch.empty((B, 2), dtype=torch.float64, **pin),
                                   target_norm=torch.empty((B, 2), dtype=torch.float64, **pin))
        return self._h_out

    def h2d_bytes_per_step(self):
        return self.num_envs

    def reset_host_counters(self):
        self._h_bytes, self._h_calls = 0, 0

    def d2h_bytes_per_step(self):
        if self._h_calls:
            return self._h_bytes / self._h_calls
        per = 3 * 8 + 8 + 1 + 1
        if self.enrich:
            per += 3 * cabi.WINDOW * cabi.WINDOW * 4 + 2 * 16
        return self.num_envs * per

    def pinned_actions(self) -> torch.Tensor:
        return torch.zeros(self.num_envs, dtype=torch.uint8, pin_memory=True)

    def step_host_packed(self, actions, decode: bool = False, chunks: Optional[int] = None):
        if self.enrich:
            raise cabi.MazeError("the packed wire format carries the -v0 observation; use step_host() with enrich=True")
        b = self.batch
        B = self.num_envs
        if chunks is None:
            chunks = 4 if B >= 262144 else 1
        if self._h_packed is None:
            self._h_packed = torch.empty(B, dtype=torch.int32, pin_memory=True)
            self._h_flag = torch.ones(1, dtype=torch.int32, pin_memory=True)
            self._h_target = torch.empty((B, 2), dtype=torch.int32, pin_memory=True)
            self._h_shape = torch.empty((B, 2), dtype=torch.int32, pin_memory=True)
            self._h_tor = torch.empty(B, dtype=torch.uint8, pin_memory=True)
            self._h_actions = torch.empty(B, dtype=torch.uint8, pin_memory=True) if self._h_actions is None else self._h_actions
            self._side_streams = [torch.cuda.Stream(self.device) for _ in range(2)]
        stream = torch.cuda.current_stream(self.device)
        mode = self._mode | cabi.STEP_PACKED | cabi.STEP_NO_WIDE
        if chunks <= 1:
            self.step(actions, extra_mode=cabi.STEP_PACKED | cabi.STEP_NO_WIDE, observe=False)
            self._h_packed.copy_(b.packed, non_blocking=True)
        else:
            if self.on_win == "regenerate":
                self.drain_regeneration()
            if isinstance(actions, torch.Tensor) and actions.device.type == "cpu" and actions.is_pinned() and actions.dtype == torch.uint8:
                src = actions.reshape(-1)
            else:
                self._h_actions.numpy()[:] = np.ascontiguousarray(actions, dtype=np.uint8).reshape(-1)
                src = self._h_actions
            start = torch.cuda.Event()
            start.record(stream)
            bounds = [B * k // chunks // 512 * 512 for k in range(chunks)] + [B]
            for k in range(chunks):
                lo, hi = bounds[k], bounds[k + 1]
                side = self._side_streams[k % 2]
                side.wait_event(start)
                with torch.cuda.stream(side):
                    self._d_actions[lo:hi].copy_(src[lo:hi], non_blocking=True)
                    b.step_view(b.view_struct(lo, hi), self._d_actions.data_ptr() + lo, mode, side.cuda_stream)
                    self._h_packed[lo:hi].copy_(b.packed[lo:hi], non_blocking=True)
            for side in self._side_streams:
                stream.wait_stream(side)
        self._h_flag.copy_(b.target_dirty, non_blocking=True)
        stream.synchronize()
        nbytes = 4 * B + 4
        if int(self._h_flag[0]) != 0:
            b.target_dirty.zero_()
            self._h_target.copy_(b.target, non_blocking=True)
            nbytes += self.num_envs * 8
            if self._h_shape_valid is False or self.grow:
                meta = self.pool.meta[b.env_maze.long()]
                self._h_shape.copy_(meta[:, :2].contiguous(), non_blocking=True)
                self._h_tor.copy_((meta[:, cabi.META_FLAGS] & cabi.FLAG_TOROIDAL).to(torch.uint8), non_blocking=True)
                nbytes += self.num_envs * (8 + 1)
                self._h_shape_valid = self._pool_is_uniform
            stream.synchronize()
        self._h_bytes += nbytes
        self._h_calls += 1
        rec = self._h_packed.numpy().view(np.uint32)
        if not decode:
            return rec
        d = cabi.decode_records(rec, self._h_shape.numpy(), self._h_tor.numpy())
        obs = {"agent": d["agent"], "target": self._h_target.numpy(), "best dir": d["best_dir"]}
        if self.reference_order:
            return obs, d["reward"], d["truncated"], d["terminated"], {}
        return obs, d["reward"], d["terminated"], d["truncated"], {}

    def step_host(self, actions: np.ndarray):
        b = self.batch
        self.step(actions)
        h = self._host_out()
        if self._h_flag is None:
            self._h_flag = torch.ones(1, dtype=torch.int32, pin_memory=True)
        self._h_flag.copy_(b.target_dirty, non_blocking=True)
        nbytes = 4
        for k in h:
            if k != "target":
                h[k].copy_(getattr(b, k), non_blocking=True)
                nbytes += h[k].numel() * h[k].element_size()
        stream = torch.cuda.current_stream(self.device)
        stream.synchronize()
        if int(self._h_flag[0]) != 0:
            b.target_dirty.zero_()
            h["target"].copy_(b.target, non_blocking=True)
            nbytes += h["target"].numel() * h["target"].element_size()
            stream.synchronize()
        self._h_bytes += nbytes
        self._h_calls += 1
        obs = {"agent": h["agent"].numpy(), "target": h["target"].numpy(), "best dir": h["best_dir"].numpy()}
        if self.enrich:
            obs.update(agent=h["agent_norm"].numpy(), target=h["target_norm"].numpy(), window=h["window"].numpy())
        term, trunc = h["terminated"].numpy().view(np.bool_), h["truncated"].numpy().view(np.bool_)
        info = {}
        if self.reference_order:
            return obs, h["reward"].numpy(), trunc, term, info
        return obs, h["reward"].numpy(), term, trunc, info

    def state_dict(self):
        return {"pool": self.pool.state_dict(), "batch": self.batch.state_dict(), "wins": self.wins}

    def load_state_dict(self, sd):
        self._drop_ahead()
        self.pool.load_state_dict(sd["pool"])
        self.batch.load_state_dict(sd["batch"])
        self.wins.copy_(sd["wins"])

    def episode_statistics(self, reduce: bool = False):
        from . import dist as mdist
        b = self.batch
        if b.stats is None:
            return None
        vec = torch.cat([b.stats.to(torch.float64), b.stats_return])
        if reduce:
            vec = mdist.reduce_statistics(vec)
        return mdist.statistics_dict(vec)

    def close(self):
        pass
```

Baseline: 44.15 billion.

## Add per-env 8-entry LRU visit cache to avoid scattered visit-count loads

Adds a small per-env cache, one 32-byte sector holding the 8 most recently visited cells and their counts. The step kernels read this cache before touching the visit array, and only spill evicted entries back to it. A state flag records whether any spill has happened, so envs that never spilled skip the array read entirely. This cuts scattered global visit loads and stores. In exchange every step adds a 32-byte cache load and store per env, more registers (hence lower launch-bound min-block counts), eviction read-before-write, and extra complexity in the observation and Q paths.

```diff
diff --git a/include/maze_b200.h b/include/maze_b200.h
--- a/include/maze_b200.h
+++ b/include/maze_b200.h
@@ -7,7 +7,7 @@
 extern "C" {
 #endif
 
-#define MAZE_ABI_VERSION 12
+#define MAZE_ABI_VERSION 13
 
 #define MAZE_E_NULL   (-1)
 #define MAZE_E_RANGE  (-2)
@@ -43,6 +43,7 @@
 #define MAZE_ST_WON         0x02
 #define MAZE_ST_MOVE_SHIFT  2
 #define MAZE_ST_NMOVES_SHIFT 4
+#define MAZE_ST_SPILLED     0x40
 
 #define MAZE_STEP_AUTORESET   0x01
 #define MAZE_STEP_WIN_NEXT    0x02
@@ -94,12 +95,13 @@
     int32_t*  target_dirty;
     uint32_t* packed;
     uint32_t* visit_bits;
-    int32_t   visit_bits_pitch;
-    int32_t   visit_bits_stride;
+    uint32_t* visit_cache;
+    int16_t   visit_bits_pitch;
+    int16_t   visit_bits_stride;
     int32_t   flags;
-    int32_t   reserved;
 } maze_env_batch;
 #define MAZE_BATCH_BORDERED 1
+#define MAZE_VISIT_CACHE_WORDS 8
 
 int  maze_sizeof(int which);
 
@@ -132,6 +134,8 @@
                    const maze_step_trace* trace, int chunk_envs, void* stream);
 
 int maze_reset(maze_ctx* ctx, const maze_env_batch* b, const uint8_t* mask, void* stream);
+
+int maze_visit_flush(maze_ctx* ctx, const maze_env_batch* b, void* stream);
 
 int maze_generate(maze_ctx* ctx, uint8_t* grids, int32_t* meta, uint8_t* table, const int32_t* ids,
                   const int32_t* count_dev, int n, int slot, int max_h, int max_w,
diff --git a/maze-solving-agent-gymnasium_b200/csrc/maze_abi.cu b/maze-solving-agent-gymnasium_b200/csrc/maze_abi.cu
--- a/maze-solving-agent-gymnasium_b200/csrc/maze_abi.cu
+++ b/maze-solving-agent-gymnasium_b200/csrc/maze_abi.cu
@@ -27,6 +27,8 @@
     if (b->visit_bits && (b->visit_bits_pitch < 1 || b->visit_bits_stride < b->visit_bits_pitch || (b->visit_bits_stride & 3) ||
                           ((uintptr_t)b->visit_bits & 15)))
         return maze_fail_arg(ctx, MAZE_E_RANGE, "visit_bits: pitch >= 1, stride a multiple of 4 words, 16-byte aligned");
+    if ((uintptr_t)b->visit_cache & 31)
+        return maze_fail_arg(ctx, MAZE_E_ALIGN, "visit_cache must be 32-byte aligned (one sector per env)");
     if (b->visit_cell_stride <= 0 || b->visit_env_stride <= 0)
         return maze_fail_arg(ctx, MAZE_E_RANGE, "visit strides (cell-major: B, 1; env-major: 1, slot)");
     if (((uintptr_t)b->meta & 15) || ((uintptr_t)b->state & 7) || ((uintptr_t)b->agent & 7) ||
diff --git a/maze-solving-agent-gymnasium_b200/csrc/maze_env.cuh b/maze-solving-agent-gymnasium_b200/csrc/maze_env.cuh
--- a/maze-solving-agent-gymnasium_b200/csrc/maze_env.cuh
+++ b/maze-solving-agent-gymnasium_b200/csrc/maze_env.cuh
@@ -98,6 +98,55 @@
 __device__ __forceinline__ void warp_clear_visits(unsigned need, const maze_env_batch& b, int e) {
     if (need & (1u << (threadIdx.x & 31)))
         for (int i = 0; i < b.visit_slot; ++i) *VISIT_AT(b, e, i) = 0;
+}
+
+constexpr int VC_K = MAZE_VISIT_CACHE_WORDS;
+struct VisitCache {
+    uint32_t w[VC_K];
+};
+
+__device__ __forceinline__ VisitCache vcache_load(const maze_env_batch& b, int e) {
+    const uint4* p = reinterpret_cast<const uint4*>(b.visit_cache + (size_t)e * VC_K);
+    const uint4 x = p[0], y = p[1];
+    VisitCache c;
+    c.w[0] = x.x; c.w[1] = x.y; c.w[2] = x.z; c.w[3] = x.w;
+    c.w[4] = y.x; c.w[5] = y.y; c.w[6] = y.z; c.w[7] = y.w;
+    return c;
+}
+__device__ __forceinline__ void vcache_store(const maze_env_batch& b, int e, const VisitCache& c) {
+    uint4* p = reinterpret_cast<uint4*>(b.visit_cache + (size_t)e * VC_K);
+    p[0] = make_uint4(c.w[0], c.w[1], c.w[2], c.w[3]);
+    p[1] = make_uint4(c.w[4], c.w[5], c.w[6], c.w[7]);
+}
+__device__ __forceinline__ void vcache_clear(VisitCache& c) {
+#pragma unroll
+    for (int i = 0; i < VC_K; ++i) c.w[i] = 0u;
+}
+__device__ __forceinline__ int vcache_find(const VisitCache& c, int n, uint32_t& hit) {
+    int pos = -1;
+    hit = 0u;
+#pragma unroll
+    for (int i = VC_K - 1; i >= 0; --i)
+        if ((c.w[i] & 0xffffu) == (unsigned)n && c.w[i] >= 0x10000u) { pos = i; hit = c.w[i]; }
+    return pos;
+}
+__device__ __forceinline__ int vcache_count(uint32_t hit, bool spilled, unsigned arr, int epoch) {
+    if (hit) return (int)(hit >> 16);
+    if (!spilled) return 0;
+    return ((int)(arr >> 8) == epoch) ? (int)(arr & 0xff) : 0;
+}
+__device__ __forceinline__ uint32_t vcache_touch(VisitCache& c, int pos, int n, int count) {
+    const int last = pos < 0 ? VC_K - 1 : pos;
+    const uint32_t victim = pos < 0 ? c.w[VC_K - 1] : 0u;
+#pragma unroll
+    for (int i = VC_K - 1; i > 0; --i)
+        if (i <= last) c.w[i] = c.w[i - 1];
+    c.w[0] = (uint32_t)n | ((uint32_t)count << 16);
+    return victim;
+}
+__device__ __forceinline__ uint16_t* vcache_slot_addr(const maze_env_batch& b, int e, uint32_t word, int W) {
+    const int n = (int)(word & 0xffffu), r = n / W;
+    return VISIT_AT(b, e, visit_index(b, r, n - r * W, W));
 }
 
 __device__ __forceinline__ void begin_episode(EnvState& s, int start, int tab_at_start, bool& wrapped) {
@@ -135,7 +184,7 @@
 };
 
 __device__ __forceinline__ StepResult env_transition(const maze_env_batch& b, int e, EnvState& st, const MazeView& mz,
-                                                     int a, const StepLuts& luts) {
+                                                     int a, const StepLuts& luts, VisitCache* vc = nullptr) {
     StepResult out = {0.0, 0, 0};
     int dr, dc;
     action_delta(a, dr, dc);
@@ -152,8 +201,16 @@
     if (inb && (tb & MAZE_TAB_OPEN)) {
         const uint64_t pol = l2_policy<MAZE_VISIT_POLICY>();
         uint16_t* vp = VISIT_AT(b, e, visit_index(b, nr, nc, mz.W));
-        const unsigned vis = visit_load(vp, pol);
-        const int cnt = ((int)(vis >> 8) == st.epoch) ? (int)(vis & 0xff) : 0;
+        bool spilled = (st.flags & MAZE_ST_SPILLED) != 0;
+        int cnt, pos = -1;
+        if (vc) {
+            uint32_t hit;
+            pos = vcache_find(*vc, idx, hit);
+            cnt = vcache_count(hit, spilled, (pos < 0 && spilled) ? visit_load(vp, pol) : 0u, st.epoch);
+        } else {
+            const unsigned vis = visit_load(vp, pol);
+            cnt = ((int)(vis >> 8) == st.epoch) ? (int)(vis & 0xff) : 0;
+        }
         if (cnt == 0) {
             if ((nr | (nc << 16)) == mz.goal) {
                 out.reward = 1.0;
@@ -165,7 +222,16 @@
         } else {
             out.reward = __ldg(luts.revisit + cnt);
         }
-        visit_store(vp, (unsigned)((st.epoch << 8) | (cnt < 255 ? cnt + 1 : 255)), pol);
+        const int next = cnt < 255 ? cnt + 1 : 255;
+        if (vc) {
+            const uint32_t victim = vcache_touch(*vc, pos, idx, next);
+            if (victim) {
+                visit_store(vcache_slot_addr(b, e, victim, mz.W), (unsigned)((st.epoch << 8) | (victim >> 16)), pol);
+                spilled = true;
+            }
+        } else {
+            visit_store(vp, (unsigned)((st.epoch << 8) | next), pol);
+        }
         visit_bit_set(b, e, nr, nc);
         st.r = nr;
         st.c = nc;
@@ -173,7 +239,7 @@
         st.consec = 0;
         int nm = (st.flags >> MAZE_ST_NMOVES_SHIFT) & 3;
         nm = nm < 2 ? nm + 1 : 2;
-        st.flags = (a << MAZE_ST_MOVE_SHIFT) | (nm << MAZE_ST_NMOVES_SHIFT);
+        st.flags = (a << MAZE_ST_MOVE_SHIFT) | (nm << MAZE_ST_NMOVES_SHIFT) | (spilled ? MAZE_ST_SPILLED : 0);
     } else {
         st.consec = st.consec < 255 ? st.consec + 1 : 255;
         out.reward = __ldg(luts.invalid + st.consec);
diff --git a/maze-solving-agent-gymnasium_b200/csrc/maze_obs.cu b/maze-solving-agent-gymnasium_b200/csrc/maze_obs.cu
--- a/maze-solving-agent-gymnasium_b200/csrc/maze_obs.cu
+++ b/maze-solving-agent-gymnasium_b200/csrc/maze_obs.cu
@@ -166,8 +166,16 @@
             const int v = open ? ((r == goal_r && c == goal_c) ? 2 : 1) : 0;
             bool trail = false;
             if (open) {
-                const unsigned vis = *VISIT_AT(b, e, visit_index(b, r, c, W));
-                const int cnt = ((int)(vis >> 8) == st.epoch) ? (int)(vis & 0xff) : 0;
+                int cnt;
+                if (b.visit_cache) {
+                    uint32_t hit;
+                    const int pos = vcache_find(vcache_load(b, e), r * W + c, hit);
+                    const bool spilled = (st.flags & MAZE_ST_SPILLED) != 0;
+                    cnt = vcache_count(hit, spilled, (pos < 0 && spilled) ? *VISIT_AT(b, e, visit_index(b, r, c, W)) : 0u, st.epoch);
+                } else {
+                    const unsigned vis = *VISIT_AT(b, e, visit_index(b, r, c, W));
+                    cnt = ((int)(vis >> 8) == st.epoch) ? (int)(vis & 0xff) : 0;
+                }
                 if (r == start_r && c == start_c) trail = has_moved;
                 else if (r == st.r && c == st.c) trail = cnt >= 2;
                 else trail = cnt >= 1;
diff --git a/maze-solving-agent-gymnasium_b200/csrc/maze_q.cu b/maze-solving-agent-gymnasium_b200/csrc/maze_q.cu
--- a/maze-solving-agent-gymnasium_b200/csrc/maze_q.cu
+++ b/maze-solving-agent-gymnasium_b200/csrc/maze_q.cu
@@ -185,6 +185,9 @@
     EnvState st = unpack_state(b.state[e]);
     int m = b.env_maze[e];
     MazeView mz = load_maze(b, m);
+    const bool has_vc = b.visit_cache != nullptr;
+    VisitCache vc;
+    if (has_vc) vc = vcache_load(b, e);
     QCursor cur = load_cursor(ag, B, e);
     double reward = 0.0;
     int term = 0, trunc = 0;
@@ -201,6 +204,7 @@
             bool wrapped;
             begin_episode(st, mz.start, __ldg(mz.tab + (mz.start & 0xffff) * mz.W + (mz.start >> 16)), wrapped);
             visit_bits_clear(b, e);
+            if (has_vc) vcache_clear(vc);
             if (wrapped)
                 for (int i = 0; i < b.visit_slot; ++i) *VISIT_AT(b, e, i) = 0;
             cur.slot = q_find_or_insert(ag, q_key(st, mz.goal, agent_id));
@@ -209,7 +213,7 @@
         }
         if (cur.slot == MAZE_Q_NO_SLOT) cur.slot = q_find_or_insert(ag, q_key(st, mz.goal, agent_id));
         const int a = q_get_action(ag, B, e, cur, nullptr);
-        const StepResult r = env_transition(b, e, st, mz, a, luts);
+        const StepResult r = env_transition(b, e, st, mz, a, luts, has_vc ? &vc : nullptr);
         reward = r.reward; term = r.term; trunc = r.trunc;
         ++n_steps;
         const uint32_t next_slot = q_find_or_insert(ag, q_key(st, mz.goal, agent_id));
@@ -225,6 +229,7 @@
     }
 
     b.state[e] = pack_state(st);
+    if (has_vc) vcache_store(b, e, vc);
     b.env_maze[e] = m;
     store_cursor(ag, B, e, cur);
     reinterpret_cast<int2*>(b.agent)[e] = make_int2(st.r, st.c);
diff --git a/maze-solving-agent-gymnasium_b200/csrc/maze_step.cu b/maze-solving-agent-gymnasium_b200/csrc/maze_step.cu
--- a/maze-solving-agent-gymnasium_b200/csrc/maze_step.cu
+++ b/maze-solving-agent-gymnasium_b200/csrc/maze_step.cu
@@ -12,9 +12,34 @@
 #ifndef MAZE_STEP_MINB2
 #define MAZE_STEP_MINB2 5
 #endif
-
-template <int EPT, bool kStats, bool kTiled>
-__global__ void __launch_bounds__(STEP_THREADS, EPT == 2 ? MAZE_STEP_MINB2 : (EPT == 1 ? MAZE_STEP_MINB1 : MAZE_STEP_MINB4))
+#ifndef MAZE_STEP_MINB1_CACHE
+#define MAZE_STEP_MINB1_CACHE 4
+#endif
+#ifndef MAZE_STEP_MINB2_CACHE
+#define MAZE_STEP_MINB2_CACHE 3
+#endif
+#ifndef MAZE_STEP_MINB4_CACHE
+#define MAZE_STEP_MINB4_CACHE 2
+#endif
+template <int EPT, bool kCache>
+constexpr int step_min_blocks() {
+    return kCache ? (EPT == 2 ? MAZE_STEP_MINB2_CACHE : (EPT == 1 ? MAZE_STEP_MINB1_CACHE : MAZE_STEP_MINB4_CACHE))
+                  : (EPT == 2 ? MAZE_STEP_MINB2 : (EPT == 1 ? MAZE_STEP_MINB1 : MAZE_STEP_MINB4));
+}
+
+#ifndef MAZE_VCACHE_EVICT
+#define MAZE_VCACHE_EVICT 1
+#endif
+#ifdef MAZE_EXP_VCACHE_CARRY
+constexpr bool kCarryOnly = true;
+#else
+constexpr bool kCarryOnly = false;
+#endif
+#ifdef MAZE_VCACHE_COUNT
+__device__ unsigned long long g_vcache_counts[4];
+#endif
+template <int EPT, bool kStats, bool kTiled, bool kCache>
+__global__ void __launch_bounds__(STEP_THREADS, (step_min_blocks<EPT, kCache>()))
 maze_step_kernel(maze_env_batch b, const uint8_t* __restrict__ actions, uint32_t mode, StepLuts luts) {
     const int base = blockIdx.x * (STEP_THREADS * EPT) + threadIdx.x;
 
@@ -22,6 +47,7 @@
     uint64_t raw[EPT];
     int m[EPT], a[EPT];
     bool valid[EPT];
+    VisitCache vc[EPT];
 #pragma unroll
     for (int k = 0; k < EPT; ++k) {
         const int e = base + k * STEP_THREADS;
@@ -30,6 +56,7 @@
         raw[k] = pol_load<MAZE_STATE_POLICY>(reinterpret_cast<const unsigned long long*>(b.state) + ee, pol_state);
         m[k] = pol_load<MAZE_STATE_POLICY>(b.env_maze + ee, pol_state);
         a[k] = __ldcs(actions + ee) & 3;
+        if (kCache) vc[k] = vcache_load(b, ee);
     }
 
     bool do_reset[EPT];
@@ -48,7 +75,8 @@
         tor[k] = __ldg(b.meta + (size_t)m[k] * MAZE_META_WORDS + MAZE_META_FLAGS) & MAZE_FLAG_TOROIDAL;
     }
 
-    int npos[EPT], idx[EPT], vidx[EPT], tb[EPT];
+    int npos[EPT], idx[EPT], vidx[EPT], tb[EPT], pos[EPT];
+    uint32_t hit[EPT];
     bool inb[EPT];
 #pragma unroll
     for (int k = 0; k < EPT; ++k) {
@@ -79,19 +107,55 @@
 #else
         tb[k] = pol_load_nc<MAZE_TABLE_POLICY>(b.table + (size_t)m[k] * b.slot + idx[k], pol_table);
 #endif
+        pos[k] = -1;
+        hit[k] = 0u;
+#ifndef MAZE_EXP_VCACHE_CARRY
+        if (kCache) pos[k] = vcache_find(vc[k], idx[k], hit[k]);
+#endif
     }
 
     const uint64_t pol = l2_policy<MAZE_VISIT_POLICY>();
     uint32_t vis[EPT];
-    bool moved[EPT];
-#pragma unroll
-    for (int k = 0; k < EPT; ++k) {
+    bool moved[EPT], spilled[EPT], from_array[EPT];
+    uint16_t* vaddr[EPT];
+#pragma unroll
+    for (int k = 0; k < EPT; ++k) {
+        const int e = base + k * STEP_THREADS;
         moved[k] = valid[k] && !do_reset[k] && inb[k] && (tb[k] & MAZE_TAB_OPEN);
+        spilled[k] = ((raw[k] >> 24) & MAZE_ST_SPILLED) != 0;
+        from_array[k] = moved[k] && (!kCache || (pos[k] < 0 && spilled[k]));
+#ifdef MAZE_EXP_VCACHE_CARRY
+        from_array[k] = moved[k];
+#endif
         vis[k] = 0;
+        vaddr[k] = nullptr;
 #ifndef MAZE_EXP_NOVISIT
-        if (moved[k]) vis[k] = visit_load(VISIT_AT(b, base + k * STEP_THREADS, vidx[k]), pol);
-#endif
-    }
+        if (from_array[k]) vis[k] = visit_load(VISIT_AT(b, e, vidx[k]), pol);
+#endif
+#ifndef MAZE_EXP_VCACHE_CARRY
+        if (kCache && moved[k] && pos[k] < 0 && vc[k].w[VC_K - 1]) {
+            vaddr[k] = vcache_slot_addr(b, e, vc[k].w[VC_K - 1], hw[k] >> 16);
+#if MAZE_VCACHE_EVICT == 1
+            (void)visit_load(vaddr[k], pol);
+#elif MAZE_VCACHE_EVICT == 2
+            asm volatile("prefetch.global.L2 [%0];" ::"l"(vaddr[k]));
+#endif
+        }
+#endif
+    }
+#ifdef MAZE_VCACHE_COUNT
+#pragma unroll
+    for (int k = 0; k < EPT; ++k) {
+        const unsigned rd = __ballot_sync(0xffffffffu, from_array[k]), wr = __ballot_sync(0xffffffffu, vaddr[k] != nullptr);
+        const unsigned mv = __ballot_sync(0xffffffffu, moved[k]), st = __ballot_sync(0xffffffffu, valid[k] && !do_reset[k]);
+        if ((threadIdx.x & 31) == 0) {
+            atomicAdd(&g_vcache_counts[0], (unsigned long long)__popc(rd));
+            atomicAdd(&g_vcache_counts[1], (unsigned long long)__popc(wr));
+            atomicAdd(&g_vcache_counts[2], (unsigned long long)__popc(mv));
+            atomicAdd(&g_vcache_counts[3], (unsigned long long)__popc(st));
+        }
+    }
+#endif
 
 #pragma unroll
     for (int k = 0; k < EPT; ++k) {
@@ -108,9 +172,11 @@
         if (do_reset[k]) {
             begin_episode(st, npos[k], tb[k], wrapped);
             visit_bits_clear(b, e);
+            if (kCache) vcache_clear(vc[k]);
         } else if (valid[k]) {
             if (moved[k]) {
-                const int cnt = ((int)(vis[k] >> 8) == st.epoch) ? (int)(vis[k] & 0xff) : 0;
+                const int cnt = kCache ? vcache_count(hit[k], spilled[k] || kCarryOnly, vis[k], st.epoch)
+                                       : (((int)(vis[k] >> 8) == st.epoch) ? (int)(vis[k] & 0xff) : 0);
                 if (cnt == 0) {
                     if (npos[k] == goal) {
                         reward = 1.0;
@@ -125,8 +191,18 @@
                     reward = __ldg(luts.revisit + cnt);
                     rcode = MAZE_REC_REWARD(MAZE_REC_KIND_REVISIT, (uint32_t)cnt);
                 }
+                const int next = cnt < 255 ? cnt + 1 : 255;
+                bool spill = spilled[k];
 #ifndef MAZE_EXP_NOVISIT
-                visit_store(VISIT_AT(b, e, vidx[k]), (unsigned)((st.epoch << 8) | (cnt < 255 ? cnt + 1 : 255)), pol);
+                if (kCache && !kCarryOnly) {
+                    const uint32_t victim = vcache_touch(vc[k], pos[k], idx[k], next);
+                    if (victim) {
+                        visit_store(vaddr[k], (unsigned)((st.epoch << 8) | (victim >> 16)), pol);
+                        spill = true;
+                    }
+                } else {
+                    visit_store(VISIT_AT(b, e, vidx[k]), (unsigned)((st.epoch << 8) | next), pol);
+                }
                 visit_bit_set(b, e, npos[k] & 0xffff, npos[k] >> 16);
 #endif
                 st.r = npos[k] & 0xffff;
@@ -135,7 +211,7 @@
                 st.consec = 0;
                 int nm = (st.flags >> MAZE_ST_NMOVES_SHIFT) & 3;
                 nm = nm < 2 ? nm + 1 : 2;
-                st.flags = (a[k] << MAZE_ST_MOVE_SHIFT) | (nm << MAZE_ST_NMOVES_SHIFT);
+                st.flags = (a[k] << MAZE_ST_MOVE_SHIFT) | (nm << MAZE_ST_NMOVES_SHIFT) | (spill ? MAZE_ST_SPILLED : 0);
             } else {
                 st.consec = st.consec < 255 ? st.consec + 1 : 255;
                 reward = __ldg(luts.invalid + st.consec);
@@ -161,6 +237,7 @@
         if (!valid[k]) continue;
 
         pol_store<MAZE_STATE_POLICY>(reinterpret_cast<unsigned long long*>(b.state) + e, (unsigned long long)pack_state(st), pol_state);
+        if (kCache && (moved[k] || do_reset[k])) vcache_store(b, e, vc[k]);
         if (do_reset[k] && (raw[k] >> 24 & MAZE_ST_WON)) {
             st_cs(reinterpret_cast<int2*>(b.target) + e, make_int2(goal & 0xffff, goal >> 16));
             if (b.target_dirty) *b.target_dirty = 1;
@@ -220,6 +297,11 @@
         const int sidx = (start & 0xffff) * W + (start >> 16);
         begin_episode(s, start, __ldg(b.table + (size_t)m * b.slot + sidx), wrapped);
         visit_bits_clear(b, ee);
+        if (b.visit_cache) {
+            VisitCache c;
+            vcache_clear(c);
+            vcache_store(b, ee, c);
+        }
     }
     const unsigned need = __ballot_sync(0xffffffffu, wrapped);
     if (need) warp_clear_visits(need, b, ee);
@@ -245,6 +327,9 @@
     EnvState st = unpack_state(b.state[e]);
     int m = b.env_maze[e];
     MazeView mz = load_maze(b, m);
+    const bool has_vc = b.visit_cache != nullptr;
+    VisitCache vc;
+    if (has_vc) vc = vcache_load(b, e);
     double reward = 0.0, ep_return = b.ep_return ? b.ep_return[e] : 0.0;
     int term = 0, trunc = 0;
     bool target_changed = false;
@@ -260,13 +345,14 @@
             bool wrapped;
             begin_episode(st, mz.start, __ldg(mz.tab + (mz.start & 0xffff) * mz.W + (mz.start >> 16)), wrapped);
             visit_bits_clear(b, e);
+            if (has_vc) vcache_clear(vc);
             if (wrapped)
                 for (int i = 0; i < b.visit_slot; ++i) *VISIT_AT(b, e, i) = 0;
             reward = 0.0; term = 0; trunc = 0;
             ep_return = 0.0;
             target_changed = true;
         } else {
-            const StepResult r = env_transition(b, e, st, mz, __ldcs(actions + (size_t)k * B + e) & 3, luts);
+            const StepResult r = env_transition(b, e, st, mz, __ldcs(actions + (size_t)k * B + e) & 3, luts, has_vc ? &vc : nullptr);
             reward = r.reward; term = r.term; trunc = r.trunc;
             ep_return += reward;
             ++n_steps;
@@ -286,6 +372,7 @@
         if (tr.truncated) __stcs(tr.truncated + at, (uint8_t)trunc);
     }
     b.state[e] = pack_state(st);
+    if (has_vc) vcache_store(b, e, vc);
     b.env_maze[e] = m;
     reinterpret_cast<int2*>(b.agent)[e] = make_int2(st.r, st.c);
     if (target_changed) {
@@ -308,7 +395,39 @@
     }
 }
 
-}
+__global__ void __launch_bounds__(STEP_THREADS)
+maze_visit_flush_kernel(maze_env_batch b) {
+    const int e = blockIdx.x * STEP_THREADS + threadIdx.x;
+    if (e >= b.num_envs) return;
+    const int epoch = unpack_state(b.state[e]).epoch;
+    const int W = __ldg(b.meta + (size_t)b.env_maze[e] * MAZE_META_WORDS + MAZE_META_W);
+    const VisitCache c = vcache_load(b, e);
+#pragma unroll
+    for (int i = 0; i < VC_K; ++i)
+        if (c.w[i]) *vcache_slot_addr(b, e, c.w[i], W) = (uint16_t)((epoch << 8) | (c.w[i] >> 16));
+}
+
+}
+
+extern "C" int maze_visit_flush(maze_ctx* ctx, const maze_env_batch* b, void* stream) {
+    if (!ctx) return MAZE_E_NULL;
+    if (int rc = maze_check_batch(ctx, b)) return rc;
+    if (!b->visit_cache) return 0;
+    maze_visit_flush_kernel<<<(b->num_envs + STEP_THREADS - 1) / STEP_THREADS, STEP_THREADS, 0, static_cast<cudaStream_t>(stream)>>>(*b);
+    MAZE_CHECK(cudaGetLastError());
+    return 0;
+}
+
+#ifdef MAZE_VCACHE_COUNT
+extern "C" int maze_vcache_debug_counts(unsigned long long* out, int reset) {
+    if (cudaMemcpyFromSymbol(out, g_vcache_counts, sizeof(g_vcache_counts)) != cudaSuccess) return -1;
+    if (reset) {
+        const unsigned long long zero[4] = {0, 0, 0, 0};
+        if (cudaMemcpyToSymbol(g_vcache_counts, zero, sizeof(zero)) != cudaSuccess) return -1;
+    }
+    return 0;
+}
+#endif
 
 extern "C" int maze_step_many(maze_ctx* ctx, const maze_env_batch* b, const uint8_t* actions, int k_steps, uint32_t mode,
                               const maze_step_trace* trace, int chunk_envs, void* stream) {
@@ -348,16 +467,21 @@
     if (b->num_envs < 64 * 1024) ept = 1;
     auto grid_for = [&](int e) { return (b->num_envs + STEP_THREADS * e - 1) / (STEP_THREADS * e); };
     auto launch = [&](auto kernel, int e) { kernel<<<grid_for(e), STEP_THREADS, 0, st>>>(*b, actions, mode, luts); };
+#define MAZE_STEP_DISPATCH_C(EPT_, C_)                                                                    \
+    do {                                                                                                  \
+        if (stats) { if (tiled) launch(maze_step_kernel<EPT_, true, true, C_>, EPT_); else launch(maze_step_kernel<EPT_, true, false, C_>, EPT_); } \
+        else       { if (tiled) launch(maze_step_kernel<EPT_, false, true, C_>, EPT_); else launch(maze_step_kernel<EPT_, false, false, C_>, EPT_); } \
+    } while (0)
 #define MAZE_STEP_DISPATCH(EPT_)                                                                          \
     do {                                                                                                  \
-        if (stats) { if (tiled) launch(maze_step_kernel<EPT_, true, true>, EPT_); else launch(maze_step_kernel<EPT_, true, false>, EPT_); } \
-        else       { if (tiled) launch(maze_step_kernel<EPT_, false, true>, EPT_); else launch(maze_step_kernel<EPT_, false, false>, EPT_); } \
+        if (cache) MAZE_STEP_DISPATCH_C(EPT_, true); else MAZE_STEP_DISPATCH_C(EPT_, false);             \
     } while (0)
-    const bool tiled = b->visit_tiled != 0;
+    const bool tiled = b->visit_tiled != 0, cache = b->visit_cache != nullptr;
     if (ept >= 4) MAZE_STEP_DISPATCH(4);
     else if (ept == 2) MAZE_STEP_DISPATCH(2);
     else MAZE_STEP_DISPATCH(1);
 #undef MAZE_STEP_DISPATCH
+#undef MAZE_STEP_DISPATCH_C
     MAZE_CHECK(cudaGetLastError());
     return 0;
 }
diff --git a/maze-solving-agent-gymnasium_b200/csrc/maze_window.cuh b/maze-solving-agent-gymnasium_b200/csrc/maze_window.cuh
--- a/maze-solving-agent-gymnasium_b200/csrc/maze_window.cuh
+++ b/maze-solving-agent-gymnasium_b200/csrc/maze_window.cuh
@@ -46,6 +46,19 @@
     m2 = openm & ~start_bit & ~seen;
 }
 
+__device__ __forceinline__ unsigned vcache_row_bits(const maze_env_batch& b, int e, int rr, int c0, int W) {
+    const VisitCache c = vcache_load(b, e);
+    unsigned bits = 0u;
+#pragma unroll
+    for (int i = 0; i < VC_K; ++i) {
+        const int d = (int)(c.w[i] & 0xffffu) - rr * W;
+        int j = d - c0;
+        j = j < 0 ? j + W : (j >= W ? j - W : j);
+        if (c.w[i] && d >= 0 && d < W && j < MAZE_WINDOW) bits |= 1u << j;
+    }
+    return bits;
+}
+
 __device__ __forceinline__ void window_row_masks(const maze_env_batch& b, int e, const EnvState& st, const MazeView& mz, int row,
                                                  unsigned& m0, unsigned& m1, unsigned& m2) {
     constexpr int WIN = MAZE_WINDOW;
@@ -81,7 +94,7 @@
             tword[k] = (4 * k - off < WIN) ? __ldg(tw + k) : 0u;
             vword[k] = (tc0 + k < wt) ? vt[(size_t)(tc0 + k) * 4] : 0ull;
         }
-        unsigned openm = 0, seen = 0;
+        unsigned openm = 0, seen = b.visit_cache ? vcache_row_bits(b, e, rr, c0, W) : 0u;
 #pragma unroll
         for (int k = 0; k < 5; ++k)
 #pragma unroll
@@ -127,4 +140,5 @@
         m1 |= ((open && idx != goal_idx) ? 1u : 0u) << j;
         m2 |= (fresh ? 1u : 0u) << j;
     }
+    if (b.visit_cache && !b.visit_bits) m2 &= ~vcache_row_bits(b, e, rr, c0, W);
 }
diff --git a/maze-solving-agent-gymnasium_b200/maze_b200/cabi.py b/maze-solving-agent-gymnasium_b200/maze_b200/cabi.py
--- a/maze-solving-agent-gymnasium_b200/maze_b200/cabi.py
+++ b/maze-solving-agent-gymnasium_b200/maze_b200/cabi.py
@@ -5,14 +5,15 @@
 
 from .build import LIB_PATH
 
-ABI_VERSION = 12
+ABI_VERSION = 13
 BATCH_BORDERED = 1
 
 META_WORDS = 8
 META_H, META_W, META_START, META_GOAL, META_MAX_STEPS, META_FLAGS, META_SOL_LEN, META_SPARE = range(8)
 FLAG_TOROIDAL = 1
 TAB_OPEN, TAB_CODE_SHIFT, TAB_D4_SHIFT = 0x01, 1, 4
-ST_NEEDS_RESET, ST_WON, ST_MOVE_SHIFT, ST_NMOVES_SHIFT = 0x01, 0x02, 2, 4
+ST_NEEDS_RESET, ST_WON, ST_MOVE_SHIFT, ST_NMOVES_SHIFT, ST_SPILLED = 0x01, 0x02, 2, 4, 0x40
+VISIT_CACHE_WORDS = 8
 STEP_AUTORESET, STEP_WIN_NEXT, STEP_WIN_QUEUE, STEP_PACKED, STEP_NO_WIDE = 0x01, 0x02, 0x04, 0x08, 0x10
 REC_CODE_SHIFT, REC_TERM_SHIFT, REC_TRUNC_SHIFT, REC_KIND_SHIFT, REC_INDEX_SHIFT = 16, 19, 20, 21, 23
 ALGO_RPRIM, ALGO_DFS, ALGO_PRIMKILL = 0, 1, 2
@@ -38,7 +39,8 @@
         ("visit_cell_stride", C.c_int64), ("visit_env_stride", C.c_int64),
         ("visit_tiled", C.c_int32), ("visit_slot", C.c_int32),
         ("target_dirty", C.c_void_p), ("packed", C.c_void_p),
-        ("visit_bits", C.c_void_p), ("visit_bits_pitch", C.c_int32), ("visit_bits_stride", C.c_int32), ("flags", C.c_int32), ("reserved", C.c_int32),
+        ("visit_bits", C.c_void_p), ("visit_cache", C.c_void_p),
+        ("visit_bits_pitch", C.c_int16), ("visit_bits_stride", C.c_int16), ("flags", C.c_int32),
     ]
 
 
@@ -108,6 +110,7 @@
     "maze_step_many": (C.c_int, [C.c_void_p, C.POINTER(MazeEnvBatch), C.c_void_p, C.c_int, C.c_uint32, C.POINTER(MazeStepTrace),
                                  C.c_int, C.c_void_p]),
     "maze_reset": (C.c_int, [C.c_void_p, C.POINTER(MazeEnvBatch), C.c_void_p, C.c_void_p]),
+    "maze_visit_flush": (C.c_int, [C.c_void_p, C.POINTER(MazeEnvBatch), C.c_void_p]),
     "maze_generate": (C.c_int, [C.c_void_p, C.c_void_p, C.c_void_p, C.c_void_p, C.c_void_p, C.c_void_p, C.c_int,
                                 C.c_int, C.c_int, C.c_int, C.c_uint64, C.c_int64, C.c_int, C.c_void_p, C.c_void_p]),
     "maze_curriculum": (C.c_int, [C.c_void_p, C.c_void_p, C.c_void_p, C.c_void_p, C.c_void_p] + [C.c_int] * 8 + [C.c_void_p]),
diff --git a/maze-solving-agent-gymnasium_b200/maze_b200/engine.py b/maze-solving-agent-gymnasium_b200/maze_b200/engine.py
--- a/maze-solving-agent-gymnasium_b200/maze_b200/engine.py
+++ b/maze-solving-agent-gymnasium_b200/maze_b200/engine.py
@@ -196,7 +196,7 @@
 class MazeBatch:
 
     def __init__(self, pool: MazePool, num_envs: int, env_maze=None, stats: bool = False, pool_stride: int = 1,
-                 queue: bool = False, visit_layout: str = "cell", visit_bits: bool = False):
+                 queue: bool = False, visit_layout: str = "cell", visit_bits: bool = False, visit_cache: bool = True):
         if visit_layout not in ("cell", "env", "tile"):
             raise ValueError("visit_layout must be 'cell', 'env' or 'tile'")
         self.visit_layout = visit_layout
@@ -234,11 +234,12 @@
         self.visit_bits_pitch = (mw + 31) // 32
         self.visit_bits_stride = _round_up(mh * self.visit_bits_pitch, 4)
         self.visit_bits = torch.zeros((B, self.visit_bits_stride), dtype=torch.int32, device=d) if visit_bits else None
+        self.visit_cache = torch.zeros((B, cabi.VISIT_CACHE_WORDS), dtype=torch.int32, device=d) if visit_cache else None
         self.pool_stride = int(pool_stride)
         self._c = self._make_struct()
 
     _CKPT = ("env_maze", "state", "visits", "agent", "target", "best_dir", "reward", "terminated", "truncated",
-             "ep_return", "stats", "stats_return", "queue", "queue_count", "target_dirty", "visit_bits")
+             "ep_return", "stats", "stats_return", "queue", "queue_count", "target_dirty", "visit_bits", "visit_cache")
 
     def state_dict(self):
         sd = {k: getattr(self, k) for k in self._CKPT if getattr(self, k) is not None}
@@ -248,6 +249,8 @@
     def load_state_dict(self, sd):
         if sd["visit_layout"] != self.visit_layout or sd["state"].shape != self.state.shape:
             raise ValueError("checkpoint was taken from a batch of another size / visit layout")
+        if ("visit_cache" in sd) != (self.visit_cache is not None):
+            raise ValueError("checkpoint was taken from a batch with%s a visit cache" % ("out" if self.visit_cache is not None else ""))
         for k in self._CKPT:
             if getattr(self, k) is not None and k in sd:
                 getattr(self, k).copy_(sd[k])
@@ -272,7 +275,8 @@
             target_dirty=self.target_dirty.data_ptr(), packed=self.packed.data_ptr(),
             visit_bits=None if self.visit_bits is None else self.visit_bits.data_ptr(),
             visit_bits_pitch=self.visit_bits_pitch, visit_bits_stride=self.visit_bits_stride,
-            flags=0 if p.any_toroidal else cabi.BATCH_BORDERED, reserved=0)
+            flags=0 if p.any_toroidal else cabi.BATCH_BORDERED,
+            visit_cache=None if self.visit_cache is None else self.visit_cache.data_ptr())
 
     def sync_flags(self):
         want = 0 if self.pool.any_toroidal else cabi.BATCH_BORDERED
@@ -292,6 +296,8 @@
         c.visits = self._c.visits + lo * self._c.visit_env_stride * 2
         if self._c.visit_bits:
             c.visit_bits = self._c.visit_bits + lo * self.visit_bits_stride * 4
+        if self._c.visit_cache:
+            c.visit_cache = self._c.visit_cache + lo * cabi.VISIT_CACHE_WORDS * 4
         return c
 
     def step_view(self, view: cabi.MazeEnvBatch, actions_ptr, mode: int, stream):
@@ -303,6 +309,10 @@
             mask = mask.to(device=self.device, dtype=torch.uint8).contiguous()
         rc = cabi.lib().maze_reset(self.ctx.handle, C.byref(self._c), cabi.ptr(mask), cabi.current_stream(self.device))
         self.ctx.check(rc, "maze_reset")
+
+    def flush_visits(self):
+        rc = cabi.lib().maze_visit_flush(self.ctx.handle, C.byref(self._c), cabi.current_stream(self.device))
+        self.ctx.check(rc, "maze_visit_flush")
 
     def step(self, actions: torch.Tensor, mode: int = 0):
         if actions.dtype != torch.uint8 or actions.device != self.device or not actions.is_contiguous():
diff --git a/maze-solving-agent-gymnasium_b200/maze_b200/vector_env.py b/maze-solving-agent-gymnasium_b200/maze_b200/vector_env.py
--- a/maze-solving-agent-gymnasium_b200/maze_b200/vector_env.py
+++ b/maze-solving-agent-gymnasium_b200/maze_b200/vector_env.py
@@ -55,7 +55,7 @@
                  on_win: str = "keep", reference_order: bool = False, stats: bool = True,
                  slot_id_base: int = 0, pool: Optional[MazePool] = None, env_maze=None, enrich: bool = False,
                  candidates: int = 1, start_shape=None, grow: int = 0, algorithm_schedule=None, visit_layout=None,
-                 regenerate_ahead: Optional[int] = None):
+                 regenerate_ahead: Optional[int] = None, visit_cache: bool = True):
         if topology not in ("euclid", "toroidal"):
             raise ValueError("topology must be 'euclid' or 'toroidal'")
         if on_win not in ("keep", "next", "regenerate"):
@@ -104,7 +104,8 @@
             per = max(1, self.num_envs // pool.num_mazes)
             env_maze = (torch.arange(self.num_envs, device=self.device, dtype=torch.int32) // per).clamp_(max=pool.num_mazes - 1)
         self.batch = MazeBatch(pool, self.num_envs, env_maze=env_maze, stats=stats, queue=(on_win == "regenerate"),
-                               visit_layout=visit_layout or ("tile" if self.enrich else "cell"), visit_bits=self.enrich)
+                               visit_layout=visit_layout or ("tile" if self.enrich else "cell"), visit_bits=self.enrich,
+                               visit_cache=visit_cache)
         self._mode = ((cabi.STEP_AUTORESET if self.autoreset else 0)
                       | (cabi.STEP_WIN_NEXT if on_win == "next" else 0)
                       | (cabi.STEP_WIN_QUEUE if on_win == "regenerate" else 0))
```

Result: slower. 36.76 billion, median of 6 (-16.7%).
